# Z2PackDev/TBmodels

Hardware: AMD Instinct MI355X
Metric: k-points/sec (H(k)+eig) at N_orb=64, N_R=4096 (higher is better)
Workload: dtype f64; 1 GPU; cfg2: dense N_orb=64 N_R=4096, 100000 random k-points per GPU, eigenval (H(k)+eig); kpoints_per_gpu=100000, collective=none, rccl_ranks=0, eigensolver=auto

## Files before the change

### include/tbk.h

```cpp
#ifndef TBK_H
#define TBK_H

#include <stdint.h>

#ifdef __cplusplus
extern "C" {
#endif

typedef struct tbk_model tbk_model;
typedef struct tbk_kdotp tbk_kdotp;
typedef struct tbk_comm tbk_comm;

typedef enum tbk_status {
    TBK_OK = 0,
    TBK_ERR_ARGUMENT = 1,
    TBK_ERR_DEVICE = 2,
    TBK_ERR_MEMORY = 3,
    TBK_ERR_NOT_FINITE = 4,
    TBK_ERR_NO_CONVERGENCE = 5
} tbk_status;

enum { TBK_EIG_AUTO = 0, TBK_EIG_WAVE = 1, TBK_EIG_ROCSOLVER = 2 };
enum {
    TBK_OPT_EIGENSOLVER = 1,
    TBK_OPT_K_CHUNK = 2,
    TBK_OPT_TIMING = 3,
    TBK_OPT_FOLD = 4
};

const char* tbk_version(void);
const char* tbk_last_error(void);
int tbk_device_count(int* count);


int tbk_model_create_dense(int device, int dim, int n_orb, int64_t n_r, const int32_t* R,
                           const double* hop, tbk_model** out);

int tbk_model_create_csr(int device, int dim, int n_orb, int64_t n_r, const int32_t* R,
                         const int64_t* r_ptr, const int32_t* row, const int32_t* col,
                         const double* val, tbk_model** out);

void tbk_model_destroy(tbk_model* m);
int tbk_model_set_option(tbk_model* m, int option, int64_t value);
int tbk_model_info(const tbk_model* m, int* device, int* dim, int* n_orb, int64_t* n_r,
                   int* is_sparse, int64_t* staged_bytes);
enum { TBK_CNT_EIGENVAL_CALLS = 0, TBK_CNT_FOLDED_CALLS = 1, TBK_CNT_FOLDED_KPOINTS = 2,
       TBK_CNT_LIBRARY_CALLS = 3,
       TBK_CNT_COUNT = 4 };
int tbk_model_counter(tbk_model* m, int counter, int64_t* value);


int tbk_hamilton(tbk_model* m, const double* k, int64_t nk, int convention, const double* pos,
                 double* H_out);

int tbk_eigenval(tbk_model* m, const double* k, int64_t nk, double* E_out);

int tbk_eigenval_multi(tbk_model* const* handles, int n_handles, const double* k, int64_t nk, double* E_out);
int tbk_hamilton_multi(tbk_model* const* handles, int n_handles, const double* k, int64_t nk, int convention,
                       const double* pos, double* H_out);

int tbk_hamilton_device(tbk_model* m, const double* d_k, int64_t nk, int convention,
                        const double* d_pos, double* d_H);
int tbk_eigenval_device(tbk_model* m, const double* d_k, int64_t nk, double* d_E);
int tbk_eigenval_device_hint(tbk_model* m, const double* d_k, const double* h_k, int64_t nk, double* d_E);
int tbk_eigenval_check(tbk_model* m);
int tbk_synchronize(tbk_model* m);

enum { TBK_REDUCE_AUTO = 0, TBK_REDUCE_ONE_STAGE = 1, TBK_REDUCE_TWO_STAGE = 2 };
int tbk_tridiagonal_reduce(int device, int n_orb, int64_t nk, const double* H, int method, double* d, double* e,
                           double* H_reduced);

int tbk_reduce_standalone(int device, int n_orb, int64_t nk, int reps, double* us_per_matrix);

int tbk_kdotp_create(int device, int dim, int n_orb, int64_t n_p, const int32_t* powers,
                     const double* coeffs, tbk_kdotp** out);
void tbk_kdotp_destroy(tbk_kdotp* m);
int tbk_kdotp_hamilton(tbk_kdotp* m, const double* k, int64_t nk, double* H_out);
int tbk_kdotp_eigenval(tbk_kdotp* m, const double* k, int64_t nk, double* E_out);
int tbk_kdotp_eigenval_multi(tbk_kdotp* const* handles, int n_handles, const double* k, int64_t nk, double* E_out);
int tbk_kdotp_hamilton_multi(tbk_kdotp* const* handles, int n_handles, const double* k, int64_t nk, double* H_out);

int tbk_kdotp_coefficients(tbk_model* m, const double* k0, int64_t n_p, const int32_t* powers,
                           const double* prefactor, double* coeffs_out);

int tbk_device_malloc(int device, int64_t bytes, void** d_ptr);
int tbk_device_free(int device, void* d_ptr);
int tbk_memcpy_h2d(int device, void* d_dst, const void* h_src, int64_t bytes);
int tbk_memcpy_d2h(int device, void* h_dst, const void* d_src, int64_t bytes);
int tbk_device_mem_info(int device, int64_t* free_bytes, int64_t* total_bytes);

enum { TBK_T_PHASE = 0, TBK_T_HK = 1, TBK_T_EIG = 2, TBK_T_QL = 3, TBK_T_COUNT = 4 };
int tbk_get_timing(tbk_model* m, double* ms, int64_t* launches, int reset);

int tbk_comm_unique_id(void* id128);
int tbk_comm_create(int device, int world_size, int rank, const void* id128, tbk_comm** out);
void tbk_comm_destroy(tbk_comm* c);
int tbk_comm_ranks(tbk_comm* c, int* count, int* rank);
int tbk_comm_allgather_f64(tbk_comm* c, tbk_model* m, const double* d_send, double* d_recv,
                           int64_t count);
int tbk_comm_allgather_f64_overlapped(tbk_comm* c, tbk_model* m, const double* d_send, double* d_recv,
                                      int64_t count, int slot);
int tbk_comm_wait_slot(tbk_comm* c, tbk_model* m, int slot);
int tbk_comm_synchronize(tbk_comm* c);
int tbk_comm_agree(tbk_comm* c, int status, double* verdict);
int tbk_comm_prepare_gather(tbk_comm* c, int n_orb, int64_t per);

int tbk_eigenval_device_gather(tbk_comm* c, tbk_model* m, const double* d_k, const double* h_k, int64_t nk, int64_t per,
                               int host_status, double* d_all, double* d_status_all);

int tbk_mfma_f64_peak(int device, double* tflops);

#ifdef __cplusplus
}
#endif
#endif
```

### tbmodels_amd/csrc/tbk_api.hip

```cpp

#include <algorithm>
#include <cmath>
#include <cstdarg>
#include <cstdlib>
#include <cstring>
#include <dlfcn.h>
#include <functional>
#include <new>
#include <vector>

#include "tbk_internal.h"

static thread_local char g_err[1024] = "";

void tbk_set_error(const char* fmt, ...) {
    va_list ap;
    va_start(ap, fmt);
    vsnprintf(g_err, sizeof(g_err), fmt, ap);
    va_end(ap);
}

extern "C" const char* tbk_last_error(void) { return g_err; }
extern "C" const char* tbk_version(void) { return "tbk 0.1 (gfx950)"; }

extern "C" int tbk_device_count(int* count) {
    TBK_ARG(count != nullptr, "count is NULL");
    int n = 0;
    hipError_t e = hipGetDeviceCount(&n);
    if (e != hipSuccess) {
        (void)hipGetLastError();
        n = 0;
    }
    *count = n;
    return TBK_OK;
}

int DevBuf::reserve(size_t want) {
    if (want <= bytes) return TBK_OK;
    release();
    const size_t rounded = (want + (size_t(1) << 20) - 1) & ~((size_t(1) << 20) - 1);
    TBK_HIP(hipMalloc(&ptr, rounded));
    bytes = rounded;
    return TBK_OK;
}

void DevBuf::release() {
    if (ptr) (void)hipFree(ptr);
    ptr = nullptr;
    bytes = 0;
}

namespace {
struct RoctxApi {
    int (*push)(const char*) = nullptr;
    int (*pop)() = nullptr;
};
const RoctxApi& roctx_api() {
    static const RoctxApi api = [] {
        RoctxApi a;
        for (const char* name : {"librocprofiler-sdk-roctx.so", "librocprofiler-sdk-roctx.so.1", "libroctx64.so"}) {
            void* h = dlopen(name, RTLD_LAZY | RTLD_GLOBAL);
            if (!h) continue;
            a.push = reinterpret_cast<int (*)(const char*)>(dlsym(h, "roctxRangePushA"));
            a.pop = reinterpret_cast<int (*)()>(dlsym(h, "roctxRangePop"));
            if (a.push && a.pop) break;
            a.push = nullptr;
            a.pop = nullptr;
        }
        return a;
    }();
    return api;
}
const char* const kStageNames[TBK_T_COUNT] = {"tbk:phase_rows", "tbk:hk_contraction", "tbk:tridiag_reduction",
                                              "tbk:tridiag_eigenvalues"};
}

void tbk_range_push(const char* name) {
    const RoctxApi& api = roctx_api();
    if (api.push) (void)api.push(name);
}

void tbk_range_pop() {
    const RoctxApi& api = roctx_api();
    if (api.pop) (void)api.pop();
}

StageTimer::StageTimer(tbk_model* m_, int stage, hipStream_t s)
    : m(m_), on(m_->timing), stream(s ? s : m_->stream) {
    ev.stage = stage;
    if (on) {
        if (hipEventCreate(&ev.start) != hipSuccess || hipEventCreate(&ev.stop) != hipSuccess) {
            on = false;
            return;
        }
        tbk_range_push(kStageNames[stage]);
        (void)hipEventRecord(ev.start, stream);
    }
}

StageTimer::~StageTimer() {
    if (on) {
        (void)hipEventRecord(ev.stop, stream);
        tbk_range_pop();
        m->events.push_back(ev);
    }
}

static inline int64_t round_up(int64_t x, int64_t q) { return (x + q - 1) / q * q; }

static int require_device(int device) {
    int n = 0;
    if (hipGetDeviceCount(&n) != hipSuccess || n == 0) {
        (void)hipGetLastError();
        tbk_set_error("no HIP device visible: libtbk has no CPU path");
        return TBK_ERR_DEVICE;
    }
    if (device < 0 || device >= n) {
        tbk_set_error("device %d out of range (have %d)", device, n);
        return TBK_ERR_ARGUMENT;
    }
    TBK_HIP(hipSetDevice(device));
    return TBK_OK;
}

static int create_common(int device, int dim, int n_orb, int64_t n_r, const int32_t* R,
                         int64_t k_rows_per_r, bool pair_diagonal, tbk_model** out) {
    TBK_ARG(out != nullptr, "out is NULL");
    *out = nullptr;
    TBK_ARG(dim >= 1 && dim <= TBK_MAX_DIM, "dim must be in [1, 8]");
    TBK_ARG(n_orb >= 1 && n_orb <= 32768, "n_orb must be in [1, 32768]");
    TBK_ARG(n_r >= 0 && n_r < (int64_t(1) << 28), "n_r out of range");
    TBK_ARG(n_r == 0 || R != nullptr || k_rows_per_r == 1, "R is NULL");
    TBK_CHECK(require_device(device));

    tbk_model* m = new (std::nothrow) tbk_model();
    if (!m) {
        tbk_set_error("out of host memory");
        return TBK_ERR_MEMORY;
    }
    m->device = device;
    {
        int cus = 0;
        if (hipDeviceGetAttribute(&cus, hipDeviceAttributeMultiprocessorCount, device) == hipSuccess && cus > 0) m->n_cu = cus;
    }
    m->dim = dim;
    m->n_orb = n_orb;
    m->n_r = n_r;
    m->k2 = round_up(n_r * k_rows_per_r, TBK_BK);
    m->n_r_pad = m->k2 / k_rows_per_r;
    m->ncol = (int)(pair_diagonal ? (int64_t)n_orb * (n_orb - 1) / 2 + (n_orb + 1) / 2 : (int64_t)n_orb * (n_orb + 1) / 2);
    m->ncol_pad = (int)round_up(m->ncol, TBK_BNP);

    int rc = TBK_OK;
    auto fail = [&](int code) {
        tbk_model_destroy(m);
        return code;
    };
#define TBK_TRY(expr)                           \
    do {                                        \
        rc = [&]() -> int {                     \
            expr;                               \
            return TBK_OK;                      \
        }();                                    \
        if (rc != TBK_OK) return fail(rc);      \
    } while (0)

    TBK_TRY(TBK_HIP(hipStreamCreateWithFlags(&m->stream, hipStreamNonBlocking)));
    TBK_TRY(TBK_HIP(hipStreamCreateWithFlags(&m->stream_eig, hipStreamNonBlocking)));
    TBK_TRY(TBK_HIP(hipStreamCreateWithFlags(&m->stream_ql, hipStreamNonBlocking)));
    for (int b = 0; b < 2; ++b) {
        TBK_TRY(TBK_HIP(hipEventCreateWithFlags(&m->ev_hk[b], hipEventDisableTiming)));
        TBK_TRY(TBK_HIP(hipEventCreateWithFlags(&m->ev_tri[b], hipEventDisableTiming)));
        TBK_TRY(TBK_HIP(hipEventCreateWithFlags(&m->ev_ql[b], hipEventDisableTiming)));
        TBK_TRY(TBK_HIP(hipEventCreateWithFlags(&m->ev_out[b], hipEventDisableTiming)));
        if (b == 0) TBK_TRY(TBK_HIP(hipEventCreateWithFlags(&m->ev_sync, hipEventDisableTiming | hipEventReleaseToSystem)));
    }
    TBK_TRY(TBK_ROCBLAS(rocblas_create_handle(&m->blas)));
    TBK_TRY(TBK_ROCBLAS(rocblas_set_stream(m->blas, m->stream)));
    TBK_TRY(TBK_CHECK(m->ws_flag.reserve(2 * sizeof(int))));
    TBK_TRY(TBK_HIP(hipMemsetAsync(m->ws_flag.ptr, 0, 2 * sizeof(int), m->stream)));
    m->h_stage_bytes = std::max<size_t>(size_t(320) << 10,
                                        n_orb <= 1024 ? (size_t)n_orb * n_orb * 16 + (size_t)n_orb * dim * 8 + (size_t(64) << 10) : 0);
    if (hipHostMalloc(&m->h_stage, m->h_stage_bytes, hipHostMallocNonCoherent) != hipSuccess) {
        (void)hipGetLastError();
        m->h_stage = nullptr;
        m->h_stage_bytes = 0;
    }

    {
        std::vector<int32_t> colmap((size_t)m->ncol_pad, -1);
        size_t e = 0;
        for (int i = 0; i < n_orb; ++i) {
            if (!pair_diagonal)
                colmap[e++] = (int32_t)((i << 16) | i);
            else if (i % 2 == 0)
                colmap[e++] = i + 1 < n_orb ? (int32_t)((i << 16) | TBK_SLOT_PAIR | (i + 1)) : (int32_t)((i << 16) | i);
            for (int j = i + 1; j < n_orb; ++j) colmap[e++] = (int32_t)((i << 16) | j);
        }
        TBK_TRY(TBK_HIP(hipMalloc((void**)&m->d_colmap, colmap.size() * sizeof(int32_t))));
        TBK_TRY(TBK_HIP(hipMemcpy(m->d_colmap, colmap.data(), colmap.size() * sizeof(int32_t),
                                  hipMemcpyHostToDevice)));
        m->staged_bytes += (int64_t)(colmap.size() * sizeof(int32_t));
    }
    if (n_r > 0 && R != nullptr && k_rows_per_r == 2) m->h_R.assign(R, R + (size_t)n_r * dim);
    if (m->n_r_pad > 0 && R != nullptr) {
        std::vector<int32_t> r_pad((size_t)m->n_r_pad * dim, 0);
        std::memcpy(r_pad.data(), R, (size_t)n_r * dim * sizeof(int32_t));
        TBK_TRY(TBK_HIP(hipMalloc((void**)&m->d_R, r_pad.size() * sizeof(int32_t))));
        TBK_TRY(TBK_HIP(hipMemcpy(m->d_R, r_pad.data(), r_pad.size() * sizeof(int32_t),
                                  hipMemcpyHostToDevice)));
        m->staged_bytes += (int64_t)(r_pad.size() * sizeof(int32_t));
    }
#undef TBK_TRY
    *out = m;
    return TBK_OK;
}

extern "C" int tbk_model_create_dense(int device, int dim, int n_orb, int64_t n_r, const int32_t* R,
                                      const double* hop, tbk_model** out) {
    TBK_ARG(out != nullptr, "out is NULL");
    *out = nullptr;
    TBK_ARG(n_r == 0 || hop != nullptr, "hop is NULL");
    tbk_model* m = nullptr;
    TBK_CHECK(create_common(device, dim, n_orb, n_r, R, 2, true, &m));
    m->sparse = false;
    int rc = TBK_OK;
    double* d_raw = nullptr;
    const size_t raw_bytes = (size_t)n_r * n_orb * n_orb * 2 * sizeof(double);
    rc = [&]() -> int {
        if (raw_bytes) {
            TBK_HIP(hipMalloc((void**)&d_raw, raw_bytes));
            TBK_HIP(hipMemcpyAsync(d_raw, hop, raw_bytes, hipMemcpyHostToDevice, m->stream));
        }
        TBK_CHECK(tbk_stage_dense(m, d_raw));
        TBK_HIP(hipStreamSynchronize(m->stream));
        return TBK_OK;
    }();
    if (d_raw) (void)hipFree(d_raw);
    if (rc != TBK_OK) {
        tbk_model_destroy(m);
        return rc;
    }
    *out = m;
    return TBK_OK;
}

extern "C" int tbk_model_create_csr(int device, int dim, int n_orb, int64_t n_r, const int32_t* R,
                                    const int64_t* r_ptr, const int32_t* row, const int32_t* col,
                                    const double* val, tbk_model** out) {
    TBK_ARG(out != nullptr, "out is NULL");
    *out = nullptr;
    TBK_ARG(n_r >= 0, "n_r out of range");
    TBK_ARG(n_r == 0 || r_ptr != nullptr, "r_ptr is NULL");
    const int64_t nnz = n_r > 0 ? r_ptr[n_r] : 0;
    TBK_ARG(n_r == 0 || r_ptr[0] == 0, "r_ptr[0] must be 0");
    TBK_ARG(nnz >= 0, "negative nnz");
    TBK_ARG(nnz == 0 || (row && col && val), "row/col/val is NULL");
    for (int64_t r = 0; r < n_r; ++r) TBK_ARG(r_ptr[r] <= r_ptr[r + 1], "r_ptr not monotone");
    for (int64_t t = 0; t < nnz; ++t)
        TBK_ARG(row[t] >= 0 && row[t] < n_orb && col[t] >= 0 && col[t] < n_orb,
                "row/col index out of range");

    tbk_model* m = nullptr;
    TBK_CHECK(create_common(device, dim, n_orb, n_r, R, 2, false, &m));
    m->sparse = true;

    auto packed_index = [n_orb](int i, int j) -> int64_t {
        return (int64_t)i * n_orb - (int64_t)i * (i - 1) / 2 + (j - i);
    };
    std::vector<int64_t> cptr((size_t)m->ncol + 1, 0);
    for (int64_t t = 0; t < nnz; ++t) {
        const int i = std::min(row[t], col[t]), j = std::max(row[t], col[t]);
        cptr[(size_t)packed_index(i, j) + 1]++;
    }
    for (int e = 0; e < m->ncol; ++e) cptr[(size_t)e + 1] += cptr[(size_t)e];
    std::vector<int32_t> rec_r((size_t)nnz);
    std::vector<double> rec_v((size_t)nnz * 2);
    {
        std::vector<int64_t> cursor(cptr.begin(), cptr.end() - 1);
        for (int64_t r = 0; r < n_r; ++r)
            for (int64_t t = r_ptr[r]; t < r_ptr[r + 1]; ++t) {
                const int i = row[t], j = col[t];
                const int kind = (i == j) ? 2 : (i < j ? 0 : 1);
                const int64_t e = packed_index(std::min(i, j), std::max(i, j));
                const int64_t slot = cursor[(size_t)e]++;
                rec_r[(size_t)slot] = (int32_t)((kind << 28) | (int32_t)r);
                rec_v[(size_t)slot * 2] = val[2 * t];
                rec_v[(size_t)slot * 2 + 1] = val[2 * t + 1];
            }
    }
    m->nnz_rec = nnz;
    int rc = [&]() -> int {
        TBK_HIP(hipMalloc((void**)&m->d_cptr, cptr.size() * sizeof(int64_t)));
        TBK_HIP(hipMemcpy(m->d_cptr, cptr.data(), cptr.size() * sizeof(int64_t), hipMemcpyHostToDevice));
        m->staged_bytes += (int64_t)(cptr.size() * sizeof(int64_t));
        if (nnz > 0) {
            TBK_HIP(hipMalloc((void**)&m->d_rec_r, (size_t)nnz * sizeof(int32_t)));
            TBK_HIP(hipMalloc((void**)&m->d_rec_v, (size_t)nnz * 2 * sizeof(double)));
            TBK_HIP(hipMemcpy(m->d_rec_r, rec_r.data(), (size_t)nnz * sizeof(int32_t), hipMemcpyHostToDevice));
            TBK_HIP(hipMemcpy(m->d_rec_v, rec_v.data(), (size_t)nnz * 2 * sizeof(double), hipMemcpyHostToDevice));
            m->staged_bytes += nnz * (int64_t)(sizeof(int32_t) + 2 * sizeof(double));
            const int kt = tbk_csr_tile_kpoints(n_r);
            if (kt > 0) {
                std::vector<int64_t> sptr;
                std::vector<int32_t> srec_r;
                std::vector<double> srec_v;
                tbk_csr_schedule(m->ncol, kt, cptr, rec_r, rec_v, sptr, srec_r, srec_v);
                m->sched_steps = sptr.back();
                auto upload = [&](void** dst, const void* src, size_t bytes) -> int {
                    TBK_HIP(hipMalloc(dst, std::max<size_t>(bytes, 8)));
                    if (bytes) TBK_HIP(hipMemcpy(*dst, src, bytes, hipMemcpyHostToDevice));
                    m->staged_bytes += (int64_t)bytes;
                    return TBK_OK;
                };
                TBK_CHECK(upload((void**)&m->d_sptr, sptr.data(), sptr.size() * sizeof(int64_t)));
                TBK_CHECK(upload((void**)&m->d_srec_r, srec_r.data(), srec_r.size() * sizeof(int32_t)));
                TBK_CHECK(upload((void**)&m->d_srec_v, srec_v.data(), srec_v.size() * sizeof(double)));
                m->sched_kt = kt;
            }
        }
        return TBK_OK;
    }();
    if (rc != TBK_OK) {
        tbk_model_destroy(m);
        return rc;
    }
    *out = m;
    return TBK_OK;
}

extern "C" void tbk_model_destroy(tbk_model* m) {
    if (!m) return;
    (void)hipSetDevice(m->device);
    hipStream_t streams[] = {m->stream, m->stream_eig, m->stream_ql, m->stream_xl[0], m->stream_xl[1], m->stream_xl[2]};
    for (hipStream_t st : streams)
        if (st) (void)hipStreamSynchronize(st);
    for (hipEvent_t e : m->ev_xl)
        if (e) (void)hipEventDestroy(e);
    for (int b = 0; b < 2; ++b) {
        if (m->ev_hk[b]) (void)hipEventDestroy(m->ev_hk[b]);
        if (m->ev_tri[b]) (void)hipEventDestroy(m->ev_tri[b]);
        if (m->ev_ql[b]) (void)hipEventDestroy(m->ev_ql[b]);
        if (m->ev_out[b]) (void)hipEventDestroy(m->ev_out[b]);
        if (b == 0 && m->ev_sync) (void)hipEventDestroy(m->ev_sync);
    }
    for (auto& ev : m->events) {
        (void)hipEventDestroy(ev.start);
        (void)hipEventDestroy(ev.stop);
    }
    if (m->blas) (void)rocblas_destroy_handle(m->blas);
    if (m->h_stage) (void)hipHostFree(m->h_stage);
    for (hipStream_t st : streams)
        if (st) (void)hipStreamDestroy(st);
    void* ptrs[] = {m->d_R, m->d_colmap, m->d_B, m->d_cptr, m->d_rec_r, m->d_rec_v, m->d_powers, m->d_sptr, m->d_srec_r, m->d_srec_v};
    for (void* p : ptrs)
        if (p) (void)hipFree(p);
    DevBuf* bufs[] = {&m->ws_phase, &m->ws_H, &m->ws_E,   &m->ws_E2,
                      &m->ws_info,  &m->ws_k, &m->ws_pos, &m->ws_out, &m->ws_out2, &m->ws_flag, &m->ws_orb, &m->ws_part, &m->ws_kfold, &m->ws_kline, &m->ws_band, &m->ws_bandmat[0], &m->ws_bandmat[1], &m->ws_H2, &m->ws_xl, &m->ws_posraw};
    for (DevBuf* b : bufs) b->release();
    tbk_fold_release(m);
    delete m;
}

extern "C" int tbk_model_set_option(tbk_model* m, int option, int64_t value) {
    TBK_ARG(m != nullptr, "model is NULL");
    TBK_LOCK(m);
    switch (option) {
        case TBK_OPT_EIGENSOLVER:
            TBK_ARG(value >= TBK_EIG_AUTO && value <= TBK_EIG_ROCSOLVER, "unknown eigensolver");
            m->eigensolver = (int)value;
            return TBK_OK;
        case TBK_OPT_K_CHUNK:
            TBK_ARG(value >= 0, "k chunk must be >= 0");
            m->k_chunk = value;
            return TBK_OK;
        case TBK_OPT_TIMING:
            m->timing = value != 0;
            return TBK_OK;
        case TBK_OPT_FOLD:
            m->fold_enabled = value != 0;
            return TBK_OK;
        default:
            tbk_set_error("unknown option %d", option);
            return TBK_ERR_ARGUMENT;
    }
}

extern "C" int tbk_model_info(const tbk_model* m, int* device, int* dim, int* n_orb, int64_t* n_r,
                              int* is_sparse, int64_t* staged_bytes) {
    TBK_ARG(m != nullptr, "model is NULL");
    if (device) *device = m->device;
    if (dim) *dim = m->dim;
    if (n_orb) *n_orb = m->n_orb;
    if (n_r) *n_r = m->n_r;
    if (is_sparse) *is_sparse = m->sparse ? 1 : 0;
    if (staged_bytes) *staged_bytes = m->staged_bytes;
    return TBK_OK;
}

static int64_t choose_chunk(tbk_model* m, int64_t nk, bool with_eig) {
    if (nk <= TBK_BM) return TBK_BM;
    const int64_t n = m->n_orb;
    int64_t per_k = m->k2 * 8 + (with_eig ? n * n * 16 + (int64_t)tbk_eig_scratch_per_k(m) : 0);
    if (per_k < 64) per_k = 64;
    size_t free_b = 0, total_b = 0;
    if (hipMemGetInfo(&free_b, &total_b) != hipSuccess) free_b = size_t(8) << 30;
    free_b += m->ws_H.bytes + m->ws_H2.bytes + m->ws_phase.bytes + m->ws_band.bytes + m->ws_bandmat[0].bytes + m->ws_bandmat[1].bytes +
              m->ws_E.bytes + m->ws_xl.bytes;
    const bool mid = n > 64 && n <= 256;
    int64_t budget = std::min<int64_t>((int64_t)(free_b / 4), int64_t(mid ? 64 : n > 64 ? 24 : 6) << 30);
    int64_t chunk = budget / per_k / TBK_BM * TBK_BM;
    int64_t cap = mid ? 131072 : 32768;
    if (n < 64) cap *= std::min<int64_t>(32, (64 / n) * (64 / n));
    chunk = std::max<int64_t>(TBK_BM, std::min<int64_t>(chunk, cap));
    if (m->k_chunk > 0) chunk = round_up(m->k_chunk, TBK_BM);
    else if (chunk >= 4096) chunk = chunk / 4096 * 4096;
    return std::min(chunk, round_up(nk, TBK_BM));
}

static inline int64_t phase_ld(int64_t nk) { return round_up(nk, TBK_BM); }

static int fill_rows(tbk_model* m, const double* d_k, int64_t nk, int64_t nk_pad, double* d_A) {
    if (m->kdotp)
        return tbk_launch_monomials(m->stream, m->d_powers, m->dim, m->n_r, m->k2, d_k, nk, nk_pad, d_A);
    return tbk_launch_phase(m, d_k, nk, nk_pad, d_A);
}

static int build_h(tbk_model* m, const double* d_A, int64_t nk, int64_t nk_pad, int mode,
                   int convention, const double* d_k, const double* d_pos, double* d_H) {
    if (m->sparse)
        return tbk_launch_hk_csr(m, d_A, nk, nk_pad, mode, convention, d_k, d_pos, d_H);
    return tbk_launch_hk_dense(m, d_A, nk, nk_pad, mode, convention, d_k, d_pos, d_H);
}

extern "C" int tbk_hamilton_device(tbk_model* m, const double* d_k, int64_t nk, int convention,
                                   const double* d_pos, double* d_H) {
    TBK_ARG(m != nullptr, "model is NULL");
    TBK_LOCK(m);
    TBK_ARG(convention == 1 || convention == 2, "convention must be 1 or 2");
    TBK_ARG(nk >= 0, "nk < 0");
    if (nk == 0) return TBK_OK;
    TBK_ARG(d_k && d_H, "k / H is NULL");
    TBK_ARG(convention == 2 || d_pos != nullptr, "convention 1 needs pos");
    TBK_HIP(hipSetDevice(m->device));
    const int64_t chunk = choose_chunk(m, nk, false);
    const size_t nn2 = (size_t)m->n_orb * m->n_orb * 2;
    for (int64_t c0 = 0; c0 < nk; c0 += chunk) {
        const int64_t nkc = std::min(chunk, nk - c0);
        const int64_t nk_pad = phase_ld(nkc);
        TBK_CHECK(m->ws_phase.reserve((size_t)std::max<int64_t>(m->k2, 1) * nk_pad * sizeof(double)));
        double* d_A = m->ws_phase.as<double>();
        const double* kc = d_k + c0 * m->dim;
        const bool own_rows = tbk_hk_inline_phases(m, nkc);
        if (!own_rows) TBK_CHECK(fill_rows(m, kc, nkc, nk_pad, d_A));
        const double* d_orb = nullptr;
        const bool inline_orb = m->h_k_inline != nullptr && m->d_pos_inline != nullptr && nk == 1 && own_rows;
        if (convention == 1 && !inline_orb) {
            TBK_CHECK(m->ws_orb.reserve((size_t)nkc * m->n_orb * 2 * sizeof(double)));
            TBK_CHECK(tbk_launch_orbital_phases(m, kc, d_pos, nkc, m->ws_orb.as<double>()));
            d_orb = m->ws_orb.as<double>();
        }
        TBK_CHECK(build_h(m, own_rows ? nullptr : d_A, nkc, nk_pad, HK_FULL, convention, kc, d_orb, d_H + (size_t)c0 * nn2));
    }
    return TBK_OK;
}

constexpr int64_t TBK_SMALL_CALL = 4096;
constexpr int64_t TBK_SMALL_CALL_PER_ORBITAL = 768;

static int launch_tridiag_eigenvalues(tbk_model* m, hipStream_t s, double* d_de, int64_t nk, double* d_E,
                                      bool beside_ql = false, bool small_call = false, const void* d_band = nullptr) {
    if (d_band) TBK_CHECK(tbk_launch_band_chase(m, s, d_band, nk, d_de));
    if (tbk_eig_small_supported(m->n_orb) && !small_call) return tbk_launch_ql(m, s, d_de, nk, d_E, beside_ql);
    return tbk_launch_bisect(m, s, d_de, nk, d_E);
}

static std::vector<int64_t> chunk_schedule(tbk_model* m, int64_t nk, int64_t chunk) {
    std::vector<int64_t> out;
    const int64_t unit = 4096;
    if (!tbk_eig_small_supported(m->n_orb) || m->k_chunk > 0 || chunk < 2 * unit || nk < 3 * unit) {
        for (int64_t c0 = 0; c0 < nk; c0 += chunk) out.push_back(std::min(chunk, nk - c0));
        return out;
    }
    const int64_t last = unit + nk % unit;
    int64_t rest = nk - last;
    const int64_t n_big = (rest + chunk - 1) / chunk;
    for (int64_t i = 0; i < n_big; ++i) {
        const int64_t share = round_up((rest + (n_big - i) - 1) / (n_big - i), unit);
        const int64_t take = std::min(std::min(share, chunk), rest);
        out.push_back(take);
        rest -= take;
    }
    out.push_back(last);
    return out;
}

using HBuilder = std::function<int(int64_t c0, int64_t nkc, double* d_H)>;

static std::vector<int64_t> run_schedule(const std::vector<int64_t>& runs, int64_t chunk) {
    std::vector<int64_t> out;
    int64_t cur = 0;
    for (size_t r = 0; r + 1 < runs.size(); ++r) {
        int64_t len = runs[r + 1] - runs[r];
        if (cur > 0 && cur + len > chunk) {
            out.push_back(cur);
            cur = 0;
        }
        while (len > chunk) {
            out.push_back(chunk);
            len -= chunk;
        }
        cur += len;
    }
    if (cur > 0) out.push_back(cur);
    return out;
}

static int eigenval_wave_pipeline(tbk_model* m, const double* d_k, int64_t nk, double* d_E, const HBuilder* builder = nullptr,
                                  const std::vector<int64_t>* runs = nullptr) {
    int64_t rows_ready_for = -1;
    const auto prepare_rows = [&](int64_t c0, int64_t nkc) -> int {
        if (tbk_hk_inline_phases(m, nkc)) return TBK_OK;
        const int64_t nk_pad = phase_ld(nkc);
        TBK_CHECK(m->ws_phase.reserve((size_t)std::max<int64_t>(m->k2, 1) * nk_pad * sizeof(double)));
        TBK_CHECK(fill_rows(m, d_k + c0 * m->dim, nkc, nk_pad, m->ws_phase.as<double>()));
        rows_ready_for = c0;
        return TBK_OK;
    };
    const HBuilder direct = [&](int64_t c0, int64_t nkc, double* d_H) -> int {
        const int64_t nk_pad = phase_ld(nkc);
        const double* kc = d_k + c0 * m->dim;
        if (tbk_hk_inline_phases(m, nkc)) return build_h(m, nullptr, nkc, nk_pad, HK_TRI, 2, kc, nullptr, d_H);
        if (rows_ready_for != c0) TBK_CHECK(prepare_rows(c0, nkc));
        return build_h(m, m->ws_phase.as<double>(), nkc, nk_pad, HK_TRI, 2, kc, nullptr, d_H);
    };
    const HBuilder& build = builder ? *builder : direct;
    const int64_t chunk = choose_chunk(m, nk, true);
    const size_t n = (size_t)m->n_orb;
    const size_t nn2 = n * n * 2;
    DevBuf* debuf[2] = {&m->ws_E, &m->ws_E2};
    const std::vector<int64_t> sched =
        (runs != nullptr && m->k_chunk == 0 && nk > chunk) ? run_schedule(*runs, chunk) : chunk_schedule(m, nk, chunk);
    const int64_t n_chunks = (int64_t)sched.size();
    const int64_t max_chunk = *std::max_element(sched.begin(), sched.end());
    const bool small_call = nk <= std::max<int64_t>(TBK_SMALL_CALL, TBK_SMALL_CALL_PER_ORBITAL * (int64_t)m->n_orb);
    TBK_CHECK(m->ws_H.reserve((size_t)max_chunk * nn2 * sizeof(double)));
    for (int b = 0; b < (n_chunks > 1 ? 2 : 1); ++b)
        TBK_CHECK(debuf[b]->reserve((size_t)max_chunk * n * 2 * sizeof(double)));
    double* d_H = m->ws_H.as<double>();
    const bool h_overlap = n_chunks > 2 && builder != nullptr && tbk_eig_small_supported(m->n_orb);
    double* d_Hbuf[2] = {d_H, d_H};
    if (h_overlap) {
        TBK_CHECK(m->ws_H2.reserve((size_t)max_chunk * nn2 * sizeof(double)));
        d_Hbuf[1] = m->ws_H2.as<double>();
    }
    const bool two_stage = !tbk_eig_small_supported(m->n_orb) && tbk_eig_two_stage(m) && n_chunks > 1 && !tbk_band_fused(m->n_orb);
    if (two_stage) {
        TBK_CHECK(m->ws_band.reserve((size_t)max_chunk * tbk_band_scratch_per_matrix(m->n_orb)));
        for (int b = 0; b < 2; ++b) TBK_CHECK(m->ws_bandmat[b].reserve((size_t)max_chunk * tbk_band_bytes_per_matrix(m->n_orb)));
        TBK_CHECK(tbk_band_xl_reserve(m, max_chunk));
    }
    if (n_chunks == 1) {
        double* d_de = debuf[0]->as<double>();
        TBK_CHECK(build(0, nk, d_H));
        if (tbk_eig_small_supported(m->n_orb))
            TBK_CHECK(tbk_launch_tridiag(m, m->stream, d_H, nk, d_de));
        else
            TBK_CHECK(tbk_launch_tridiag_stream(m, m->stream, d_H, nk, d_de));
        TBK_CHECK(launch_tridiag_eigenvalues(m, m->stream, d_de, nk, d_E, false, small_call));
        if (m->chunk_done) {
            TBK_HIP(hipEventRecord(m->ev_ql[0], m->stream));
            TBK_CHECK(m->chunk_done(0, nk, m->ev_ql[0]));
        }
        return TBK_OK;
    }
    int64_t prev_c0 = 0, prev_nkc = 0, c0 = 0;
    for (int64_t c = 0; c < n_chunks; ++c) {
        const int b = (int)(c & 1);
        const int64_t nkc = sched[c];
        double* d_de = debuf[b]->as<double>();
        d_H = d_Hbuf[b];
        if (c >= 1) {
            if (!builder) TBK_CHECK(prepare_rows(c0, nkc));
            if (!h_overlap)
                TBK_HIP(hipStreamWaitEvent(m->stream, m->ev_tri[b ^ 1], 0));
            else if (c >= 2)
                TBK_HIP(hipStreamWaitEvent(m->stream, m->ev_tri[b], 0));
            if (c >= 2 && !h_overlap) TBK_HIP(hipStreamWaitEvent(m->stream, m->ev_ql[b], 0));
        }
        TBK_CHECK(build(c0, nkc, d_H));
        TBK_HIP(hipEventRecord(m->ev_hk[b], m->stream));

        TBK_HIP(hipStreamWaitEvent(m->stream_eig, m->ev_hk[b], 0));
        if (c >= 2 && h_overlap) TBK_HIP(hipStreamWaitEvent(m->stream_eig, m->ev_ql[b], 0));
        if (tbk_eig_small_supported(m->n_orb))
            TBK_CHECK(tbk_launch_tridiag(m, m->stream_eig, d_H, nkc, d_de));
        else if (two_stage)
            TBK_CHECK(tbk_launch_band_reduce(m, m->stream_eig, d_H, nkc, m->ws_band.ptr, m->ws_bandmat[b].ptr));
        else
            TBK_CHECK(tbk_launch_tridiag_stream(m, m->stream_eig, d_H, nkc, d_de));
        TBK_HIP(hipEventRecord(m->ev_tri[b], m->stream_eig));

        if (c >= 1) {
            TBK_HIP(hipStreamWaitEvent(m->stream_ql, m->ev_hk[b], 0));
            if (h_overlap) TBK_HIP(hipStreamWaitEvent(m->stream_ql, m->ev_tri[b ^ 1], 0));
            TBK_CHECK(launch_tridiag_eigenvalues(m, m->stream_ql, debuf[b ^ 1]->as<double>(), prev_nkc,
                                                 d_E + (size_t)prev_c0 * n, false, small_call,
                                                 two_stage ? m->ws_bandmat[b ^ 1].ptr : nullptr));
            TBK_HIP(hipEventRecord(m->ev_ql[b ^ 1], m->stream_ql));
            if (m->chunk_done) TBK_CHECK(m->chunk_done(prev_c0, prev_nkc, m->ev_ql[b ^ 1]));
        }
        prev_c0 = c0;
        prev_nkc = nkc;
        c0 += nkc;
    }
    {
        const int b = (int)((n_chunks - 1) & 1);
        TBK_CHECK(launch_tridiag_eigenvalues(m, m->stream_eig, debuf[b]->as<double>(), prev_nkc,
                                             d_E + (size_t)prev_c0 * n, n_chunks > 1,
                                             small_call || n_chunks > 1, two_stage ? m->ws_bandmat[b].ptr : nullptr));
        TBK_HIP(hipEventRecord(m->ev_ql[b], m->stream_eig));
        if (m->chunk_done) TBK_CHECK(m->chunk_done(prev_c0, prev_nkc, m->ev_ql[b]));
    }
    for (int b = 0; b < (n_chunks > 1 ? 2 : 1); ++b) TBK_HIP(hipStreamWaitEvent(m->stream, m->ev_ql[b], 0));
    TBK_HIP(hipStreamWaitEvent(m->stream, m->ev_tri[(n_chunks - 1) & 1], 0));
    return TBK_OK;
}

static int eigenval_folded(tbk_model* m, const double* d_k, const double* h_k, int64_t nk, double* d_E, bool* done) {
    *done = false;
    if (!m->fold_enabled || m->sparse || m->kdotp || m->dim < 2 || m->n_r < 64 || nk < 1024) return TBK_OK;
    if (h_k == nullptr) return TBK_OK;
    std::vector<int64_t> runs;
    const int f = tbk_fold_choose(m, h_k, nk, runs);
    if (f < 0) return TBK_OK;
    const int dim = m->dim;
    TBK_CHECK(m->ws_kfold.reserve((size_t)nk * (dim - 1) * sizeof(double)));
    double* d_k2 = m->ws_kfold.as<double>();
    TBK_CHECK(tbk_fold_drop_component(m, d_k, dim, f, nk, d_k2));
    const size_t nn2 = (size_t)m->n_orb * m->n_orb * 2;
    const int64_t n_runs = (int64_t)runs.size() - 1;
    const int group = tbk_fold_group_size();
    int64_t group_lo = -1;
    tbk_fold_plan_t& plan1 = m->fold[f];
    std::vector<int> reduced;
    for (int d = 0; d < dim; ++d)
        if (d != f) reduced.push_back(d);

    auto piece_plane = [&](int64_t lo, int64_t hi, double* d_Hp) -> int {
        const int64_t len = hi - lo, nk_pad = phase_ld(len);
        TBK_CHECK(m->ws_phase.reserve((size_t)std::max<int64_t>(m->k2, 1) * nk_pad * sizeof(double)));
        TBK_CHECK(fill_rows(m, d_k2 + lo * (dim - 1), len, nk_pad, m->ws_phase.as<double>()));
        return build_h(m, m->ws_phase.as<double>(), len, nk_pad, HK_TRI, 2, d_k2 + lo * (dim - 1), nullptr, d_Hp);
    };

    struct LineInfo {
        bool ok = false;
        int e2 = -1;
        int64_t L = 0;
        int64_t body = 0;
        int64_t n_lines = 0;
    };
    const int dim1 = dim - 1;
    const int line_cap = 512;
    auto same_line = [&](int64_t a0, int64_t b0, int64_t L, int e2) {
        for (int64_t t = 0; t < L; ++t)
            for (int e = 0; e < dim1; ++e)
                if (e != e2 && h_k[(a0 + t) * dim + reduced[e]] != h_k[(b0 + t) * dim + reduced[e]]) return false;
        return true;
    };
    auto analyse = [&](int64_t lo, int64_t hi) -> LineInfo {
        LineInfo li;
        if (dim1 < 2 || hi - lo < 512) return li;
        int e2 = -1;
        int64_t best_changes = hi - lo;
        for (int e = 0; e < dim1; ++e) {
            int64_t changes = 0;
            for (int64_t i = lo + 1; i < hi; ++i) changes += h_k[i * dim + reduced[e]] != h_k[(i - 1) * dim + reduced[e]];
            if (changes < best_changes) {
                best_changes = changes;
                e2 = e;
            }
        }
        if (e2 < 0 || best_changes < 4) return li;
        const int c2 = reduced[e2];
        std::vector<int64_t> sb(1, lo);
        for (int64_t i = lo + 1; i < hi; ++i)
            if (h_k[i * dim + c2] != h_k[(i - 1) * dim + c2]) sb.push_back(i);
        sb.push_back(hi);
        const size_t n_sub = sb.size() - 1;
        if (n_sub < 6) return li;
        const int64_t L = sb[2] - sb[1];
        if (L < 8 || L > TBK_BM) return li;
        size_t first = (sb[1] - sb[0] == L && same_line(sb[0], sb[1], L, e2)) ? 0 : 1, last = first;
        while (last < n_sub && sb[last + 1] - sb[last] == L && same_line(sb[first], sb[last], L, e2)) ++last;
        li.n_lines = (int64_t)(last - first);
        if (li.n_lines < 4) return li;
        li.ok = true;
        li.e2 = e2;
        li.L = L;
        li.body = sb[first];
        return li;
    };
    auto fold_body = [&](tbk_fold_plan_t& plan2, const LineInfo& li, int64_t a0, int64_t n, int slot0) -> int {
        return tbk_fold_lines(m, plan2, d_k2 + a0 * dim1 + li.e2, li.L * dim1, (int)n, slot0);
    };
    auto contract_lines = [&](tbk_fold_plan_t& plan2, const LineInfo& li, int64_t a0, int64_t n, double* d_Hp) -> int {
        const int64_t row_len = (int64_t)m->ncol_pad * 2;
        tbk_fold_saved_t saved2;
        TBK_CHECK(tbk_fold_enter(m, plan2, 0, saved2));
        int rc = m->ws_kline.reserve((size_t)li.L * std::max(dim1 - 1, 1) * sizeof(double));
        if (rc == TBK_OK) rc = tbk_fold_drop_component(m, d_k2 + a0 * dim1, dim1, li.e2, li.L, m->ws_kline.as<double>());
        if (rc == TBK_OK) rc = m->ws_phase.reserve((size_t)std::max<int64_t>(m->k2, 1) * TBK_BM * sizeof(double));
        if (rc == TBK_OK) rc = fill_rows(m, m->ws_kline.as<double>(), li.L, TBK_BM, m->ws_phase.as<double>());
        if (rc == TBK_OK)
            rc = tbk_launch_hk_dense_lines(m, m->ws_phase.as<double>(), n, (int)li.L, plan2.k2 * row_len, d_Hp);
        tbk_fold_leave(m, saved2);
        return rc;
    };

    auto piece = [&](int64_t lo, int64_t hi, double* d_Hp) -> int {
        const LineInfo li = analyse(lo, hi);
        if (!li.ok) return piece_plane(lo, hi, d_Hp);
        tbk_fold_plan_t* plan2 = nullptr;
        TBK_CHECK(tbk_fold_subplan(m, plan1, li.e2, line_cap, &plan2));
        if (!plan2 || plan2->n_rho * 3 > plan1.n_rho) return piece_plane(lo, hi, d_Hp);

        if (li.body > lo) TBK_CHECK(piece_plane(lo, li.body, d_Hp));
        for (int64_t l0 = 0; l0 < li.n_lines; l0 += line_cap) {
            const int64_t nl = std::min<int64_t>(line_cap, li.n_lines - l0);
            const int64_t a0 = li.body + l0 * li.L;
            TBK_CHECK(fold_body(*plan2, li, a0, nl, 0));
            TBK_CHECK(contract_lines(*plan2, li, a0, nl, d_Hp + (size_t)(a0 - lo) * nn2));
        }
        const int64_t body_end = li.body + li.n_lines * li.L;
        if (body_end < hi) TBK_CHECK(piece_plane(body_end, hi, d_Hp + (size_t)(body_end - lo) * nn2));
        return TBK_OK;
    };

    auto enter_run = [&](size_t r, tbk_fold_saved_t& saved) -> int {
        if (group_lo < 0 || (int64_t)r < group_lo || (int64_t)r >= group_lo + group) {
            group_lo = (int64_t)r;
            const int n_g = (int)std::min<int64_t>(group, n_runs - group_lo);
            double kf[64];
            for (int g = 0; g < n_g; ++g) kf[g] = h_k[runs[(size_t)(group_lo + g)] * dim + f];
            TBK_CHECK(tbk_fold_group(m, plan1, kf, n_g, 0));
        }
        return tbk_fold_enter(m, plan1, (int)((int64_t)r - group_lo), saved);
    };
    auto batched = [&](int64_t c0, int64_t nkc, double* d_H, bool* done) -> int {
        *done = false;
        const size_t r0 = (size_t)(std::upper_bound(runs.begin(), runs.end(), c0) - runs.begin()) - 1;
        if (runs[r0] != c0) return TBK_OK;
        size_t r1 = r0;
        while (r1 + 1 < runs.size() && runs[r1 + 1] <= c0 + nkc) ++r1;
        if (r1 - r0 < 2 || runs[r1] != c0 + nkc) return TBK_OK;
        const LineInfo li0 = analyse(runs[r0], runs[r0 + 1]);
        if (!li0.ok || li0.body != runs[r0] || li0.body + li0.n_lines * li0.L != runs[r0 + 1]) return TBK_OK;
        int64_t total = li0.n_lines;
        for (size_t r = r0 + 1; r < r1; ++r) {
            const LineInfo li = analyse(runs[r], runs[r + 1]);
            if (!li.ok || li.e2 != li0.e2 || li.L != li0.L || li.body != runs[r] ||
                li.body + li.n_lines * li.L != runs[r + 1] || !same_line(runs[r0], runs[r], li0.L, li0.e2))
                return TBK_OK;
            total += li.n_lines;
        }
        if (total > line_cap) return TBK_OK;
        tbk_fold_plan_t* plan2 = nullptr;
        TBK_CHECK(tbk_fold_subplan(m, plan1, li0.e2, line_cap, &plan2));
        if (!plan2 || plan2->n_rho * 3 > plan1.n_rho) return TBK_OK;
        int slot = 0;
        for (size_t r = r0; r < r1; ++r) {
            tbk_fold_saved_t saved;
            TBK_CHECK(enter_run(r, saved));
            const int64_t n = (runs[r + 1] - runs[r]) / li0.L;
            const int rc = fold_body(*plan2, li0, runs[r], n, slot);
            tbk_fold_leave(m, saved);
            TBK_CHECK(rc);
            slot += (int)n;
        }
        {
            tbk_fold_saved_t saved;
            TBK_CHECK(enter_run(r1 - 1, saved));
            const int rc = contract_lines(*plan2, li0, c0, total, d_H);
            tbk_fold_leave(m, saved);
            TBK_CHECK(rc);
        }
        *done = true;
        return TBK_OK;
    };

    const HBuilder folded = [&](int64_t c0, int64_t nkc, double* d_H) -> int {
        {
            bool done = false;
            TBK_CHECK(batched(c0, nkc, d_H, &done));
            if (done) return TBK_OK;
        }
        size_t r = (size_t)(std::upper_bound(runs.begin(), runs.end(), c0) - runs.begin()) - 1;
        for (int64_t lo = c0; lo < c0 + nkc; ++r) {
            const int64_t hi = std::min(runs[r + 1], c0 + nkc);
            tbk_fold_saved_t saved;
            TBK_CHECK(enter_run(r, saved));
            const int rc = piece(lo, hi, d_H + (size_t)(lo - c0) * nn2);
            tbk_fold_leave(m, saved);
            TBK_CHECK(rc);
            lo = hi;
        }
        return TBK_OK;
    };
    TBK_CHECK(eigenval_wave_pipeline(m, d_k, nk, d_E, &folded, &runs));
    m->counters[TBK_CNT_FOLDED_CALLS] += 1;
    m->counters[TBK_CNT_FOLDED_KPOINTS] += nk;
    *done = true;
    return TBK_OK;
}

static bool eigenval_own_solvers(const tbk_model* m) {
    return m->eigensolver != TBK_EIG_ROCSOLVER &&
           (tbk_eig_small_supported(m->n_orb) || (m->eigensolver == TBK_EIG_AUTO && tbk_eig_stream_supported(m->n_orb)));
}

static int eigenval_device_solve(tbk_model* m, const double* d_k, const double* h_k, int64_t nk, double* d_E) {
    TBK_ARG(m != nullptr, "model is NULL");
    TBK_LOCK(m);
    TBK_ARG(nk >= 0, "nk < 0");
    if (nk == 0) return TBK_OK;
    TBK_ARG(d_k && d_E, "k / E is NULL");
    TBK_HIP(hipSetDevice(m->device));
    m->call_nk = nk;
    m->counters[TBK_CNT_EIGENVAL_CALLS] += 1;
    if (m->eigensolver == TBK_EIG_WAVE && !tbk_eig_small_supported(m->n_orb)) {
        tbk_set_error("TBK_EIG_WAVE handles n_orb <= 64 only (n_orb = %d)", m->n_orb);
        return TBK_ERR_ARGUMENT;
    }
    if (eigenval_own_solvers(m)) {
        bool done = false;
        TBK_CHECK(eigenval_folded(m, d_k, h_k, nk, d_E, &done));
        if (done) return TBK_OK;
        return eigenval_wave_pipeline(m, d_k, nk, d_E);
    }

    int64_t chunk = choose_chunk(m, nk, true);
    const size_t nn2 = (size_t)m->n_orb * m->n_orb * 2;
    chunk = std::max<int64_t>(1, std::min<int64_t>(chunk, (int64_t(1) << 29) / std::max<int64_t>(1, (int64_t)m->n_orb * m->n_orb)));
    m->counters[TBK_CNT_LIBRARY_CALLS] += 1;
    for (int64_t c0 = 0; c0 < nk; c0 += chunk) {
        const int64_t nkc = std::min(chunk, nk - c0);
        const int64_t nk_pad = phase_ld(nkc);
        TBK_CHECK(m->ws_phase.reserve((size_t)std::max<int64_t>(m->k2, 1) * nk_pad * sizeof(double)));
        TBK_CHECK(m->ws_H.reserve((size_t)nkc * nn2 * sizeof(double)));
        double* d_A = m->ws_phase.as<double>();
        double* d_H = m->ws_H.as<double>();
        const double* kc = d_k + c0 * m->dim;
        TBK_CHECK(fill_rows(m, kc, nkc, nk_pad, d_A));
        TBK_CHECK(build_h(m, d_A, nkc, nk_pad, HK_TRI, 2, kc, nullptr, d_H));
        TBK_CHECK(tbk_eig_batched(m, d_H, nkc, d_E + (size_t)c0 * m->n_orb));
    }
    return TBK_OK;
}

__global__ void __launch_bounds__(256) flag_nonfinite_kernel(const double* __restrict__ E, int64_t total, int* __restrict__ flag) {
    bool bad = false;
    for (int64_t i = (int64_t)blockIdx.x * 256 + threadIdx.x; i < total; i += (int64_t)gridDim.x * 256) bad |= !isfinite(E[i]);
    if (__any(bad) && (threadIdx.x & 63) == 0) atomicAdd(flag, 1);
}

static int eigenval_device_impl(tbk_model* m, const double* d_k, const double* h_k, int64_t nk, double* d_E) {
    TBK_CHECK(eigenval_device_solve(m, d_k, h_k, nk, d_E));
    const bool own_solvers = m != nullptr && eigenval_own_solvers(m);
    if (nk > 0 && m != nullptr && !own_solvers) {
        const int64_t total = nk * m->n_orb;
        const unsigned blocks = (unsigned)std::min<int64_t>((total + 255) / 256, 8 * 1024);
        hipLaunchKernelGGL(flag_nonfinite_kernel, dim3(blocks), dim3(256), 0, m->stream, d_E, total, m->ws_flag.as<int>() + 1);
        TBK_HIP(hipGetLastError());
    }
    return TBK_OK;
}

extern "C" int tbk_eigenval_device(tbk_model* m, const double* d_k, int64_t nk, double* d_E) {
    return eigenval_device_impl(m, d_k, nullptr, nk, d_E);
}

extern "C" int tbk_eigenval_device_hint(tbk_model* m, const double* d_k, const double* h_k, int64_t nk, double* d_E) {
    return eigenval_device_impl(m, d_k, h_k, nk, d_E);
}

extern "C" int tbk_model_counter(tbk_model* m, int counter, int64_t* value) {
    TBK_ARG(m != nullptr && value != nullptr, "model / value is NULL");
    TBK_ARG(counter >= 0 && counter < TBK_CNT_COUNT, "unknown counter");
    TBK_LOCK(m);
    *value = m->counters[counter];
    return TBK_OK;
}

static int wait_main_stream(tbk_model* m) {
    TBK_HIP(hipEventRecord(m->ev_sync, m->stream));
    TBK_HIP(hipEventSynchronize(m->ev_sync));
    return TBK_OK;
}

extern "C" int tbk_synchronize(tbk_model* m) {
    TBK_ARG(m != nullptr, "model is NULL");
    TBK_LOCK(m);
    TBK_HIP(hipSetDevice(m->device));
    return wait_main_stream(m);
}

extern "C" int tbk_eigenval_check(tbk_model* m) {
    TBK_ARG(m != nullptr, "model is NULL");
    TBK_LOCK(m);
    TBK_HIP(hipSetDevice(m->device));
    int flag[2] = {0, 0};
    TBK_HIP(hipMemcpyAsync(flag, m->ws_flag.ptr, sizeof(flag), hipMemcpyDeviceToHost, m->stream));
    TBK_HIP(hipMemsetAsync(m->ws_flag.ptr, 0, sizeof(flag), m->stream));
    TBK_CHECK(wait_main_stream(m));
    if (flag[1] != 0) {
        tbk_set_error("array must not contain infs or NaNs");
        return TBK_ERR_NOT_FINITE;
    }
    if (flag[0] != 0) {
        tbk_set_error("eigensolver did not converge for %d matrices", flag[0]);
        return TBK_ERR_NO_CONVERGENCE;
    }
    return TBK_OK;
}

extern "C" int tbk_hamilton(tbk_model* m, const double* k, int64_t nk, int convention,
                            const double* pos, double* H_out) {
    TBK_ARG(m != nullptr, "model is NULL");
    TBK_LOCK(m);
    TBK_ARG(convention == 1 || convention == 2, "convention must be 1 or 2");
    TBK_ARG(nk >= 0, "nk < 0");
    if (nk == 0) return TBK_OK;
    TBK_ARG(k && H_out, "k / H is NULL");
    TBK_ARG(convention == 2 || pos != nullptr, "convention 1 needs pos");
    TBK_HIP(hipSetDevice(m->device));
    const size_t nn2 = (size_t)m->n_orb * m->n_orb * 2;
    {
        const size_t k_bytes = (size_t)nk * m->dim * sizeof(double), h_bytes = (size_t)nk * nn2 * sizeof(double);
        const size_t p_bytes = convention == 1 ? (size_t)m->n_orb * m->dim * sizeof(double) : 0;
        const size_t h_off = (k_bytes + p_bytes + 63) / 64 * 64;
        if (m->h_stage != nullptr && h_off + h_bytes <= m->h_stage_bytes) {
            char* st = static_cast<char*>(m->h_stage);
            TBK_CHECK(m->ws_k.reserve(k_bytes));
            TBK_CHECK(m->ws_out.reserve(h_bytes));
            const bool inline_k = nk == 1 && !m->sparse && !m->kdotp && tbk_hk_inline_phases(m, 1);
            const double* d_pos = nullptr;
            if (inline_k) {
                if (convention == 1) {
                    const size_t n_pos = (size_t)m->n_orb * m->dim;
                    if (m->pos_cache.size() != n_pos || std::memcmp(m->pos_cache.data(), pos, p_bytes) != 0) {
                        TBK_CHECK(m->ws_posraw.reserve(p_bytes));
                        std::memcpy(st + k_bytes, pos, p_bytes);
                        TBK_HIP(hipMemcpyAsync(m->ws_posraw.ptr, st + k_bytes, p_bytes, hipMemcpyHostToDevice, m->stream));
                        m->pos_cache.assign(pos, pos + n_pos);
                    }
                    m->d_pos_inline = m->ws_posraw.as<double>();
                    d_pos = m->d_pos_inline;
                }
                m->h_k_inline = k;
            } else {
                std::memcpy(st, k, k_bytes);
                TBK_HIP(hipMemcpyAsync(m->ws_k.ptr, st, k_bytes, hipMemcpyHostToDevice, m->stream));
                if (convention == 1) {
                    TBK_CHECK(m->ws_pos.reserve(p_bytes));
                    std::memcpy(st + k_bytes, pos, p_bytes);
                    TBK_HIP(hipMemcpyAsync(m->ws_pos.ptr, st + k_bytes, p_bytes, hipMemcpyHostToDevice, m->stream));
                    d_pos = m->ws_pos.as<double>();
                }
            }
            constexpr size_t ZERO_COPY_MAX = size_t(1) << 20;
            const bool direct = h_bytes <= ZERO_COPY_MAX;
            double* d_out = direct ? reinterpret_cast<double*>(st + h_off) : m->ws_out.as<double>();
            const int rc_inline = tbk_hamilton_device(m, m->ws_k.as<double>(), nk, convention, d_pos, d_out);
            m->h_k_inline = nullptr;
            m->d_pos_inline = nullptr;
            TBK_CHECK(rc_inline);
            if (!direct) TBK_HIP(hipMemcpyAsync(st + h_off, m->ws_out.ptr, h_bytes, hipMemcpyDeviceToHost, m->stream));
            TBK_CHECK(wait_main_stream(m));
            std::memcpy(H_out, st + h_off, h_bytes);
            return TBK_OK;
        }
    }
    const size_t total_bytes = (size_t)nk * nn2 * sizeof(double);
    const size_t chunk_bytes = std::min<size_t>(size_t(128) << 20, std::max<size_t>(size_t(16) << 20, total_bytes / 4));
    int64_t out_chunk = std::max<int64_t>(1, (int64_t)(chunk_bytes / (nn2 * sizeof(double))));
    out_chunk = std::min(out_chunk, nk);
    const int64_t n_chunks = (nk + out_chunk - 1) / out_chunk;
    TBK_CHECK(m->ws_k.reserve((size_t)nk * m->dim * sizeof(double)));
    TBK_HIP(hipMemcpyAsync(m->ws_k.ptr, k, (size_t)nk * m->dim * sizeof(double), hipMemcpyHostToDevice, m->stream));
    const double* d_pos = nullptr;
    if (convention == 1) {
        TBK_CHECK(m->ws_pos.reserve((size_t)m->n_orb * m->dim * sizeof(double)));
        TBK_HIP(hipMemcpyAsync(m->ws_pos.ptr, pos, (size_t)m->n_orb * m->dim * sizeof(double),
                               hipMemcpyHostToDevice, m->stream));
        d_pos = m->ws_pos.as<double>();
    }
    DevBuf* obuf[2] = {&m->ws_out, &m->ws_out2};
    for (int b = 0; b < (n_chunks > 1 ? 2 : 1); ++b) TBK_CHECK(obuf[b]->reserve((size_t)out_chunk * nn2 * sizeof(double)));
    auto compute = [&](int64_t c) -> int {
        const int64_t c0 = c * out_chunk, nkc = std::min(out_chunk, nk - c0);
        TBK_CHECK(tbk_hamilton_device(m, m->ws_k.as<double>() + c0 * m->dim, nkc, convention, d_pos, obuf[c & 1]->as<double>()));
        TBK_HIP(hipEventRecord(m->ev_out[c & 1], m->stream));
        return TBK_OK;
    };
    TBK_CHECK(compute(0));
    for (int64_t c = 0; c < n_chunks; ++c) {
        const int64_t c0 = c * out_chunk, nkc = std::min(out_chunk, nk - c0);
        if (c + 1 < n_chunks) TBK_CHECK(compute(c + 1));
        TBK_HIP(hipEventSynchronize(m->ev_out[c & 1]));
        TBK_HIP(hipMemcpy(H_out + (size_t)c0 * nn2, obuf[c & 1]->ptr, (size_t)nkc * nn2 * sizeof(double), hipMemcpyDeviceToHost));
    }
    return wait_main_stream(m);
}

__global__ void __launch_bounds__(256) export_small_kernel(const double* __restrict__ E, int64_t count, const int* __restrict__ flag,
                                                           double* __restrict__ host_E, int* __restrict__ host_flag) {
    for (int64_t i = (int64_t)blockIdx.x * 256 + threadIdx.x; i < count; i += (int64_t)gridDim.x * 256) host_E[i] = E[i];
    if (blockIdx.x == 0 && threadIdx.x < 2) host_flag[threadIdx.x] = flag[threadIdx.x];
}

extern "C" int tbk_eigenval(tbk_model* m, const double* k, int64_t nk, double* E_out) {
    TBK_ARG(m != nullptr, "model is NULL");
    TBK_LOCK(m);
    TBK_ARG(nk >= 0, "nk < 0");
    if (nk == 0) return TBK_OK;
    TBK_ARG(k && E_out, "k / E is NULL");
    TBK_HIP(hipSetDevice(m->device));
    const size_t k_bytes = (size_t)nk * m->dim * sizeof(double), e_bytes = (size_t)nk * m->n_orb * sizeof(double);
    TBK_CHECK(m->ws_k.reserve(k_bytes));
    TBK_CHECK(m->ws_out.reserve(e_bytes));
    const size_t e_off = (k_bytes + 63) / 64 * 64;
    if (m->h_stage != nullptr && e_off + e_bytes + 16 <= m->h_stage_bytes) {
        char* st = static_cast<char*>(m->h_stage);
        int* flag = reinterpret_cast<int*>(st + e_off + e_bytes);
        const bool inline_k = nk == 1 && !m->sparse && !m->kdotp && eigenval_own_solvers(m) && tbk_hk_inline_phases(m, 1);
        if (inline_k) {
            m->h_k_inline = k;
        } else {
            std::memcpy(st, k, k_bytes);
            TBK_HIP(hipMemcpyAsync(m->ws_k.ptr, st, k_bytes, hipMemcpyHostToDevice, m->stream));
        }
        const int rc_inline = eigenval_device_impl(m, m->ws_k.as<double>(), k, nk, m->ws_out.as<double>());
        m->h_k_inline = nullptr;
        TBK_CHECK(rc_inline);
        {
            const int64_t count = nk * m->n_orb;
            const unsigned blocks = (unsigned)std::min<int64_t>((count + 255) / 256, 64);
            hipLaunchKernelGGL(export_small_kernel, dim3(blocks), dim3(256), 0, m->stream, m->ws_out.as<double>(), count,
                               m->ws_flag.as<int>(), reinterpret_cast<double*>(st + e_off), flag);
            TBK_HIP(hipGetLastError());
        }
        TBK_CHECK(wait_main_stream(m));
        std::memcpy(E_out, st + e_off, e_bytes);
        if (flag[0] != 0 || flag[1] != 0) return tbk_eigenval_check(m);
        return TBK_OK;
    }
    TBK_HIP(hipMemcpyAsync(m->ws_k.ptr, k, k_bytes, hipMemcpyHostToDevice, m->stream));
    TBK_CHECK(eigenval_device_impl(m, m->ws_k.as<double>(), k, nk, m->ws_out.as<double>()));
    TBK_HIP(hipMemcpyAsync(E_out, m->ws_out.ptr, e_bytes, hipMemcpyDeviceToHost, m->stream));
    return tbk_eigenval_check(m);
}

extern "C" int tbk_tridiagonal_reduce(int device, int n_orb, int64_t nk, const double* H, int method, double* d, double* e,
                                      double* H_reduced) {
    TBK_ARG(nk >= 0, "nk < 0");
    TBK_ARG(n_orb >= 1 && (n_orb <= 64 || tbk_eig_stream_supported(n_orb)),
            "n_orb must be in [1, 4096] (larger matrices go through rocSOLVER as a whole)");
    TBK_ARG(method >= TBK_REDUCE_AUTO && method <= TBK_REDUCE_TWO_STAGE, "unknown reduction method");
    TBK_ARG(method != TBK_REDUCE_TWO_STAGE || tbk_eig_band_supported(n_orb), "the two-stage reduction handles 64 < n_orb <= 4096");
    TBK_ARG(method != TBK_REDUCE_ONE_STAGE || n_orb <= 512, "the one-stage reduction handles n_orb <= 512");
    if (nk == 0) return TBK_OK;
    TBK_ARG(H && d && e, "H / d / e is NULL");
    tbk_model* m = nullptr;
    TBK_CHECK(create_common(device, 1, n_orb, 0, nullptr, 2, false, &m));
    const size_t n = (size_t)n_orb, mat_bytes = n * n * 2 * sizeof(double);
    int rc = [&]() -> int {
        TBK_LOCK(m);
        m->call_nk = nk;
        TBK_CHECK(m->ws_H.reserve((size_t)nk * mat_bytes));
        TBK_CHECK(m->ws_E.reserve((size_t)nk * n * 2 * sizeof(double)));
        TBK_HIP(hipMemcpyAsync(m->ws_H.ptr, H, (size_t)nk * mat_bytes, hipMemcpyHostToDevice, m->stream));
        if (tbk_eig_small_supported(n_orb))
            TBK_CHECK(tbk_launch_tridiag(m, m->stream, m->ws_H.as<double>(), nk, m->ws_E.as<double>()));
        else
            TBK_CHECK(tbk_launch_tridiag_stream(m, m->stream, m->ws_H.as<double>(), nk, m->ws_E.as<double>(), method));
        TBK_HIP(hipMemcpyAsync(d, m->ws_E.ptr, (size_t)nk * n * sizeof(double), hipMemcpyDeviceToHost, m->stream));
        TBK_HIP(hipMemcpyAsync(e, m->ws_E.as<double>() + (size_t)nk * n, (size_t)nk * n * sizeof(double), hipMemcpyDeviceToHost,
                               m->stream));
        if (H_reduced)
            TBK_HIP(hipMemcpyAsync(H_reduced, m->ws_H.ptr, (size_t)nk * mat_bytes, hipMemcpyDeviceToHost, m->stream));
        TBK_HIP(hipStreamSynchronize(m->stream));
        return TBK_OK;
    }();
    tbk_model_destroy(m);
    return rc;
}

__global__ void __launch_bounds__(256) random_hermitian_kernel(double* __restrict__ H, int n, int64_t nk) {
    const int64_t total = nk * (int64_t)n * n;
    for (int64_t t = (int64_t)blockIdx.x * 256 + threadIdx.x; t < total; t += (int64_t)gridDim.x * 256) {
        const int64_t mat = t / ((int64_t)n * n);
        const int r = (int)((t / n) % n), c = (int)(t % n);
        const int i = r < c ? r : c, j = r < c ? c : r;
        uint64_t x = (uint64_t)mat * 0x9E3779B97F4A7C15ull + (uint64_t)i * 0xBF58476D1CE4E5B9ull + (uint64_t)j * 0x94D049BB133111EBull + 1;
        x ^= x >> 30; x *= 0xBF58476D1CE4E5B9ull; x ^= x >> 27; x *= 0x94D049BB133111EBull; x ^= x >> 31;
        const double re = (double)(int64_t)(x >> 11) * (1.0 / 9007199254740992.0) - 0.5;
        x ^= x >> 29; x *= 0x9E3779B97F4A7C15ull; x ^= x >> 32;
        const double im = (double)(int64_t)(x >> 11) * (1.0 / 9007199254740992.0) - 0.5;
        H[2 * t] = re;
        H[2 * t + 1] = i == j ? 0.0 : (r < c ? im : -im);
    }
}

extern "C" int tbk_reduce_standalone(int device, int n_orb, int64_t nk, int reps, double* us_per_matrix) {
    TBK_ARG(us_per_matrix != nullptr, "us_per_matrix is NULL");
    TBK_ARG(nk >= 1 && reps >= 1, "nk / reps < 1");
    TBK_ARG(n_orb >= 1 && (n_orb <= 64 || tbk_eig_stream_supported(n_orb)), "n_orb must be in [1, 4096]");
    for (int q = 0; q < 3; ++q) us_per_matrix[q] = 0.0;
    tbk_model* m = nullptr;
    TBK_CHECK(create_common(device, 1, n_orb, 0, nullptr, 2, false, &m));
    const size_t n = (size_t)n_orb, mat_bytes = n * n * 2 * sizeof(double);
    DevBuf pristine;
    hipEvent_t ev[2] = {nullptr, nullptr};
    int rc = [&]() -> int {
        TBK_LOCK(m);
        m->call_nk = nk;
        TBK_CHECK(pristine.reserve((size_t)nk * mat_bytes));
        TBK_CHECK(m->ws_H.reserve((size_t)nk * mat_bytes));
        TBK_CHECK(m->ws_E.reserve((size_t)nk * n * 2 * sizeof(double)));
        TBK_HIP(hipEventCreate(&ev[0]));
        TBK_HIP(hipEventCreate(&ev[1]));
        hipLaunchKernelGGL(random_hermitian_kernel, dim3(4096), dim3(256), 0, m->stream, pristine.as<double>(), n_orb, nk);
        TBK_HIP(hipGetLastError());
        const bool band = !tbk_eig_small_supported(n_orb) && tbk_eig_two_stage(m);
        if (band) {
            TBK_CHECK(m->ws_band.reserve((size_t)nk * tbk_band_scratch_per_matrix(n_orb)));
            TBK_CHECK(m->ws_bandmat[0].reserve((size_t)nk * tbk_band_bytes_per_matrix(n_orb)));
        }
        for (int what = 0; what < (band ? 3 : 1); ++what) {
            float sum = 0.0f;
            for (int r = 0; r <= reps; ++r) {
                if (what != 2)
                    TBK_HIP(hipMemcpyAsync(m->ws_H.ptr, pristine.ptr, (size_t)nk * mat_bytes, hipMemcpyDeviceToDevice, m->stream));
                TBK_HIP(hipEventRecord(ev[0], m->stream));
                if (what == 0) {
                    if (tbk_eig_small_supported(n_orb))
                        TBK_CHECK(tbk_launch_tridiag(m, m->stream, m->ws_H.as<double>(), nk, m->ws_E.as<double>()));
                    else
                        TBK_CHECK(tbk_launch_tridiag_stream(m, m->stream, m->ws_H.as<double>(), nk, m->ws_E.as<double>(), TBK_REDUCE_AUTO));
                } else if (what == 1) {
                    TBK_CHECK(tbk_launch_band_reduce(m, m->stream, m->ws_H.as<double>(), nk, m->ws_band.ptr, m->ws_bandmat[0].ptr));
                } else {
                    TBK_CHECK(tbk_launch_band_chase(m, m->stream, m->ws_bandmat[0].ptr, nk, m->ws_E.as<double>()));
                }
                TBK_HIP(hipEventRecord(ev[1], m->stream));
                TBK_HIP(hipEventSynchronize(ev[1]));
                float ms = 0.0f;
                TBK_HIP(hipEventElapsedTime(&ms, ev[0], ev[1]));
                if (r > 0) sum += ms;
            }
            us_per_matrix[what] = (double)sum / reps * 1e3 / (double)nk;
        }
        return TBK_OK;
    }();
    for (auto& e : ev)
        if (e) (void)hipEventDestroy(e);
    pristine.release();
    tbk_model_destroy(m);
    return rc;
}

extern "C" int tbk_kdotp_create(int device, int dim, int n_orb, int64_t n_p, const int32_t* powers,
                                const double* coeffs, tbk_kdotp** out) {
    TBK_ARG(out != nullptr, "out is NULL");
    *out = nullptr;
    TBK_ARG(n_p == 0 || (powers && coeffs), "powers / coeffs is NULL");
    for (int64_t t = 0; t < n_p * dim; ++t) TBK_ARG(powers[t] >= 0, "negative power");
    tbk_model* m = nullptr;
    TBK_CHECK(create_common(device, dim, n_orb, n_p, nullptr, 1, false, &m));
    m->kdotp = true;
    double* d_raw = nullptr;
    const size_t raw_bytes = (size_t)n_p * n_orb * n_orb * 2 * sizeof(double);
    int rc = [&]() -> int {
        if (n_p > 0) {
            TBK_HIP(hipMalloc((void**)&m->d_powers, (size_t)n_p * dim * sizeof(int32_t)));
            TBK_HIP(hipMemcpy(m->d_powers, powers, (size_t)n_p * dim * sizeof(int32_t), hipMemcpyHostToDevice));
            TBK_HIP(hipMalloc((void**)&d_raw, raw_bytes));
            TBK_HIP(hipMemcpyAsync(d_raw, coeffs, raw_bytes, hipMemcpyHostToDevice, m->stream));
        }
        TBK_CHECK(tbk_stage_kdotp(m, d_raw));
        TBK_HIP(hipStreamSynchronize(m->stream));
        return TBK_OK;
    }();
    if (d_raw) (void)hipFree(d_raw);
    if (rc != TBK_OK) {
        tbk_model_destroy(m);
        return rc;
    }
    tbk_kdotp* kp = new (std::nothrow) tbk_kdotp();
    if (!kp) {
        tbk_model_destroy(m);
        tbk_set_error("out of host memory");
        return TBK_ERR_MEMORY;
    }
    kp->core = m;
    *out = kp;
    return TBK_OK;
}

extern "C" void tbk_kdotp_destroy(tbk_kdotp* kp) {
    if (!kp) return;
    tbk_model_destroy(kp->core);
    delete kp;
}

extern "C" int tbk_kdotp_hamilton(tbk_kdotp* kp, const double* k, int64_t nk, double* H_out) {
    TBK_ARG(kp != nullptr, "model is NULL");
    return tbk_hamilton(kp->core, k, nk, 2, nullptr, H_out);
}

extern "C" int tbk_kdotp_eigenval(tbk_kdotp* kp, const double* k, int64_t nk, double* E_out) {
    TBK_ARG(kp != nullptr, "model is NULL");
    return tbk_eigenval(kp->core, k, nk, E_out);
}

extern "C" int tbk_device_malloc(int device, int64_t bytes, void** d_ptr) {
    TBK_ARG(d_ptr != nullptr && bytes >= 0, "bad malloc arguments");
    TBK_CHECK(require_device(device));
    *d_ptr = nullptr;
    if (bytes == 0) return TBK_OK;
    TBK_HIP(hipMalloc(d_ptr, (size_t)bytes));
    return TBK_OK;
}

extern "C" int tbk_device_free(int device, void* d_ptr) {
    if (!d_ptr) return TBK_OK;
    TBK_CHECK(require_device(device));
    TBK_HIP(hipFree(d_ptr));
    return TBK_OK;
}

extern "C" int tbk_memcpy_h2d(int device, void* d_dst, const void* h_src, int64_t bytes) {
    TBK_CHECK(require_device(device));
    if (bytes > 0) {
        TBK_HIP(hipMemcpy(d_dst, h_src, (size_t)bytes, hipMemcpyHostToDevice));
        TBK_HIP(hipDeviceSynchronize());
    }
    return TBK_OK;
}

extern "C" int tbk_memcpy_d2h(int device, void* h_dst, const void* d_src, int64_t bytes) {
    TBK_CHECK(require_device(device));
    if (bytes > 0) TBK_HIP(hipMemcpy(h_dst, d_src, (size_t)bytes, hipMemcpyDeviceToHost));
    return TBK_OK;
}

extern "C" int tbk_device_mem_info(int device, int64_t* free_bytes, int64_t* total_bytes) {
    TBK_CHECK(require_device(device));
    size_t f = 0, t = 0;
    TBK_HIP(hipMemGetInfo(&f, &t));
    if (free_bytes) *free_bytes = (int64_t)f;
    if (total_bytes) *total_bytes = (int64_t)t;
    return TBK_OK;
}

extern "C" int tbk_get_timing(tbk_model* m, double* ms, int64_t* launches, int reset) {
    TBK_ARG(m != nullptr, "model is NULL");
    TBK_LOCK(m);
    TBK_HIP(hipSetDevice(m->device));
    TBK_HIP(hipStreamSynchronize(m->stream));
    TBK_HIP(hipStreamSynchronize(m->stream_eig));
    TBK_HIP(hipStreamSynchronize(m->stream_ql));
    for (auto& ev : m->events) {
        float t = 0.f;
        if (hipEventElapsedTime(&t, ev.start, ev.stop) == hipSuccess) {
            m->t_ms[ev.stage] += (double)t;
            m->t_n[ev.stage] += 1;
        }
        (void)hipEventDestroy(ev.start);
        (void)hipEventDestroy(ev.stop);
    }
    m->events.clear();
    for (int i = 0; i < TBK_T_COUNT; ++i) {
        if (ms) ms[i] = m->t_ms[i];
        if (launches) launches[i] = m->t_n[i];
        if (reset) {
            m->t_ms[i] = 0.0;
            m->t_n[i] = 0;
        }
    }
    return TBK_OK;
}

extern "C" int tbk_mfma_f64_peak(int device, double* tflops) {
    TBK_ARG(tflops != nullptr, "tflops is NULL");
    TBK_CHECK(require_device(device));
    return tbk_run_mfma_f64_peak(tflops);
}
```

### tbmodels_amd/csrc/tbk_hk_dense.hip

```cpp

#include <algorithm>
#include <cstdlib>
#include <type_traits>

#include "tbk_internal.h"

namespace {

typedef double d4 __attribute__((ext_vector_type(4)));
typedef double d2 __attribute__((ext_vector_type(2)));
typedef __attribute__((address_space(1))) const void* gptr_t;
typedef __attribute__((address_space(3))) void* lptr_t;

constexpr int LDA = TBK_BM + 16;
constexpr int LDB = 2 * TBK_BNP + 16;
constexpr int STAGE_DOUBLES = TBK_BK * (LDA + LDB);

static_assert(TBK_BM == 128 && TBK_BNP == 64 && TBK_BK == 16, "wave decomposition is written for 128x64x16");

struct HkArgs {
    const double* A;
    const double* Bt;
    const int32_t* colmap;
    const double* kpts;
    const int32_t* R;
    int64_t n_r;
    const double* pos;
    double* H;
    int64_t k2;
    int64_t nk;
    int64_t nk_pad;
    int ncol_pad;
    int n_orb;
    int dim;
    int mt_count;
    int nt_count;
    int xcd_rows;
    double* P;
    int splits;
    int unit_grid;
    int64_t p_rows;
    int64_t a_tile_stride;
    int64_t b_tile_stride;
    int rows_per_tile;
    int block_offset;
    int p_tiles;
    int sub_splits;
    double* P2;
    double k_val[TBK_MAX_DIM];
    int k_inline;
    const double* pos_raw;
};

__device__ __forceinline__ double hk_kcomp(const HkArgs& a, int64_t kq, int d) { return a.k_inline ? a.k_val[d] : a.kpts[kq * a.dim + d]; }

template <int MODE, int CONV>
__device__ __forceinline__ void store_element(const HkArgs& a, int64_t kq, int oi, int oj, double re, double im) {
    if (CONV == 1 && oi != oj) {
        d2 ei, ej;
        if (a.k_inline) {
            double di = 0.0, dj = 0.0;
            for (int d = 0; d < a.dim; ++d) {
                di = fma(a.k_val[d], a.pos_raw[oi * a.dim + d], di);
                dj = fma(a.k_val[d], a.pos_raw[oj * a.dim + d], dj);
            }
            double sn, cs;
            sincospi(2.0 * di, &sn, &cs);
            ei = (d2){cs, sn};
            sincospi(2.0 * dj, &sn, &cs);
            ej = (d2){cs, sn};
        } else {
            ei = *reinterpret_cast<const d2*>(a.pos + ((size_t)kq * a.n_orb + oi) * 2);
            ej = *reinterpret_cast<const d2*>(a.pos + ((size_t)kq * a.n_orb + oj) * 2);
        }
        const double cs = ei[0] * ej[0] + ei[1] * ej[1], sn = ei[0] * ej[1] - ei[1] * ej[0];
        const double t = re * cs - im * sn;
        im = re * sn + im * cs;
        re = t;
    }
    double* hk = a.H + (size_t)kq * a.n_orb * a.n_orb * 2;
    *reinterpret_cast<d2*>(hk + ((size_t)oi * a.n_orb + oj) * 2) = (d2){re, im};
    if (MODE == HK_FULL && oi != oj) *reinterpret_cast<d2*>(hk + ((size_t)oj * a.n_orb + oi) * 2) = (d2){re, -im};
}

template <int MODE, int CONV>
__device__ __forceinline__ void store_slot(const HkArgs& a, int64_t kq, int32_t slot, double v0, double v1) {
    const int oi = slot >> 16, oj = slot & 0x7fff;
    if (slot & TBK_SLOT_PAIR) {
        double* hk = a.H + (size_t)kq * a.n_orb * a.n_orb * 2;
        *reinterpret_cast<d2*>(hk + ((size_t)oi * a.n_orb + oi) * 2) = (d2){v0, 0.0};
        *reinterpret_cast<d2*>(hk + ((size_t)oj * a.n_orb + oj) * 2) = (d2){v1, 0.0};
        return;
    }
    store_element<MODE, CONV>(a, kq, oi, oj, v0, v1);
}

__device__ __forceinline__ bool tile_of_block(const HkArgs& a, int b, int& mt, int& nt) {
    if (a.xcd_rows == 0) {
        nt = b % a.nt_count;
        mt = b / a.nt_count;
        return mt < a.mt_count;
    }
    const int x = b & 7;
    const int t = b >> 3;
    const int base = a.mt_count >> 3, extra = a.mt_count & 7;
    const int rows = base + (x < extra ? 1 : 0);
    if (t >= rows * a.nt_count) return false;
    const int start = x * base + (x < extra ? x : extra);
    const int full = rows / a.xcd_rows;
    const int per_group = a.xcd_rows * a.nt_count;
    int row;
    if (t < full * per_group) {
        const int g = t / per_group, r = t % per_group;
        row = g * a.xcd_rows + r % a.xcd_rows;
        nt = r / a.xcd_rows;
    } else {
        const int tt = t - full * per_group, rr = rows - full * a.xcd_rows;
        row = full * a.xcd_rows + tt % rr;
        nt = tt / rr;
    }
    mt = start + row;
    return true;
}

template <int MODE, int CONV, bool SPLIT>
__global__ void __launch_bounds__(256, 2) hk_dense_kernel(const HkArgs a) {
    extern __shared__ __attribute__((aligned(16))) double smem[];

    const int unit = (int)blockIdx.x + a.block_offset;
    const int split_y = SPLIT ? unit / a.unit_grid : 0;
    int mt_idx, nt_idx;
    if (!tile_of_block(a, SPLIT ? unit - split_y * a.unit_grid : unit, mt_idx, nt_idx)) return;

    const int tid = threadIdx.x;
    const int lane = tid & 63;
    const int wave = __builtin_amdgcn_readfirstlane(tid >> 6);
    const int wm = wave >> 1;
    const int wn = wave & 1;
    const int l15 = lane & 15;
    const int l4 = lane >> 4;

    const int64_t m0 = (int64_t)mt_idx * a.rows_per_tile;
    const int64_t n0 = (int64_t)nt_idx * TBK_BNP;

    d4 acc[4][2][2];
#pragma unroll
    for (int i = 0; i < 4; ++i)
#pragma unroll
        for (int j = 0; j < 2; ++j)
#pragma unroll
            for (int p = 0; p < 2; ++p) acc[i][j][p] = (d4){0.0, 0.0, 0.0, 0.0};

    int s_begin = 0, n_stage = (int)(a.k2 / TBK_BK);
    if (SPLIT) {
        const int per = (n_stage + a.splits - 1) / a.splits;
        s_begin = min(split_y * per, n_stage);
        n_stage = min(s_begin + per, n_stage);
        if (a.p_tiles > 0) {
            const int per2 = (n_stage - s_begin + a.sub_splits - 1) / a.sub_splits;
            s_begin = min(s_begin + (int)blockIdx.y * per2, n_stage);
            n_stage = min(s_begin + per2, n_stage);
        }
    }

    const uint32_t lane_bytes = (uint32_t)lane * 16u;
    const int64_t ldgA = a.nk_pad * (int64_t)sizeof(double);
    const int64_t ldgB = (int64_t)a.ncol_pad * 2 * (int64_t)sizeof(double);
    const char* rowA = reinterpret_cast<const char*>(a.A + (int64_t)mt_idx * a.a_tile_stride) + ((int64_t)s_begin * TBK_BK + wave) * ldgA;
    const char* rowB = reinterpret_cast<const char*>(a.Bt + (int64_t)mt_idx * a.b_tile_stride + n0 * 2) + ((int64_t)s_begin * TBK_BK + wave) * ldgB;
    auto issue_stage = [&](auto bufc) {
        constexpr int buf = decltype(bufc)::value;
        double* sA = smem + buf * STAGE_DOUBLES + wave * LDA;
        double* sB = smem + buf * STAGE_DOUBLES + TBK_BK * LDA + wave * LDB;
        uint32_t off = lane_bytes;
        asm volatile("" : "+v"(off));
#pragma unroll
        for (int i = 0; i < 4; ++i) {
            __builtin_amdgcn_global_load_lds((gptr_t)(rowA + (int64_t)(4 * i) * ldgA + off), (lptr_t)(sA + 4 * i * LDA), 16, 0, 0);
            __builtin_amdgcn_global_load_lds((gptr_t)(rowB + (int64_t)(4 * i) * ldgB + off), (lptr_t)(sB + 4 * i * LDB), 16, 0, 0);
        }
        rowA += TBK_BK * ldgA;
        rowB += TBK_BK * ldgB;
    };
    typedef __attribute__((address_space(3))) const double* lds_cptr;
    uint32_t fragA[2][TBK_BK / 4], fragB[2][TBK_BK / 4];
    {
        const uint32_t s0 = (uint32_t)(uintptr_t)(lptr_t)smem;
#pragma unroll
        for (int buf = 0; buf < 2; ++buf)
#pragma unroll
            for (int ks = 0; ks < TBK_BK / 4; ++ks) {
                fragA[buf][ks] = s0 + 8u * (uint32_t)(buf * STAGE_DOUBLES + wm * 64 + l15 + (ks * 4 + l4) * LDA);
                fragB[buf][ks] = s0 + 8u * (uint32_t)(buf * STAGE_DOUBLES + TBK_BK * LDA + wn * 64 + l15 + (ks * 4 + l4) * LDB);
                asm volatile("" : "+v"(fragA[buf][ks]), "+v"(fragB[buf][ks]));
            }
    }
    struct Frags {
        double fa[4], fb[2][2];
    };
    auto read_frags = [&](auto bufc, auto ksc) -> Frags {
        constexpr int buf = decltype(bufc)::value, ks = decltype(ksc)::value;
        const lds_cptr sA = (lds_cptr)(uintptr_t)fragA[buf][ks];
        const lds_cptr sB = (lds_cptr)(uintptr_t)fragB[buf][ks];
        Frags f;
#pragma unroll
        for (int i = 0; i < 4; ++i) f.fa[i] = sA[i * 16];
#pragma unroll
        for (int j = 0; j < 2; ++j) {
            f.fb[j][0] = sB[j * 32];
            f.fb[j][1] = sB[j * 32 + 16];
        }
        return f;
    };
    auto mfma_step = [&](const Frags& f) {
#pragma unroll
        for (int i = 0; i < 4; ++i)
#pragma unroll
            for (int j = 0; j < 2; ++j) {
                acc[i][j][0] = __builtin_amdgcn_mfma_f64_16x16x4f64(f.fa[i], f.fb[j][0], acc[i][j][0], 0, 0, 0);
                acc[i][j][1] = __builtin_amdgcn_mfma_f64_16x16x4f64(f.fa[i], f.fb[j][1], acc[i][j][1], 0, 0, 0);
            }
    };
    using buf0 = std::integral_constant<int, 0>;
    using buf1 = std::integral_constant<int, 1>;
    using ks0 = std::integral_constant<int, 0>;
    using ks1 = std::integral_constant<int, 1>;
    using ks2 = std::integral_constant<int, 2>;
    using ks3 = std::integral_constant<int, 3>;
    static_assert(TBK_BK == 16, "four K steps per stage are written out below");
    auto stage = [&](auto bufc, auto nextc, Frags& cur, bool more) {
        Frags f1 = read_frags(bufc, ks1{});
        mfma_step(cur);
        Frags f2 = read_frags(bufc, ks2{});
        mfma_step(f1);
        Frags f3 = read_frags(bufc, ks3{});
        mfma_step(f2);
        __syncthreads();
        if (more) cur = read_frags(nextc, ks0{});
        mfma_step(f3);
    };

    const int left = n_stage - s_begin;
    if (left > 0) issue_stage(buf0{});
    __syncthreads();
    Frags cur = read_frags(buf0{}, ks0{});
    for (int pair = 0; pair < (left >> 1); ++pair) {
        issue_stage(buf1{});
        stage(buf0{}, buf1{}, cur, true);
        const bool more = 2 * pair + 2 < left;
        if (more) issue_stage(buf0{});
        stage(buf1{}, buf0{}, cur, more);
    }
    if (left & 1) stage(buf0{}, buf1{}, cur, false);

#pragma unroll
    for (int j = 0; j < 2; ++j) {
        const int e = (int)n0 + (wn * 2 + j) * 16 + l15;
        const int32_t ij = a.colmap[e];
        if (ij < 0) continue;
#pragma unroll
        for (int i = 0; i < 4; ++i) {
#pragma unroll
            for (int r = 0; r < 4; ++r) {
                const int local = wm * 64 + i * 16 + l4 + 4 * r;
                const int64_t kq = m0 + local;
                if (local >= a.rows_per_tile || kq >= a.nk) continue;
                if (SPLIT) {
                    double* part =
                        a.p_tiles > 0
                            ? a.P2 + ((((size_t)blockIdx.y * a.p_tiles + blockIdx.x) * TBK_BM + local) * TBK_BNP +
                                      (wn * 2 + j) * 16 + l15) * 2
                            : a.P + (((size_t)split_y * a.p_rows + kq) * a.ncol_pad + e) * 2;
                    *reinterpret_cast<d2*>(part) = (d2){acc[i][j][0][r], acc[i][j][1][r]};
                } else {
                    store_slot<MODE, CONV>(a, kq, ij, acc[i][j][0][r], acc[i][j][1][r]);
                }
            }
        }
    }
}

constexpr int GEMV_U = 8;

template <int NKV, bool INLINE_PHASES>
__global__ void __launch_bounds__(256) hk_gemv_kernel(const HkArgs a, int strip_doubles) {
    extern __shared__ __attribute__((aligned(16))) double s_rows[];
    constexpr int U = NKV >= 32 ? 4 : GEMV_U;
    const int lane = threadIdx.x & 63;
    const int wave = __builtin_amdgcn_readfirstlane(threadIdx.x >> 6);
    const int nblk = a.ncol_pad >> 6;
    const int b = (int)blockIdx.x, n_wg = (int)gridDim.x;
    const int xcd = b & 7, per_xcd = n_wg >> 3, extra = n_wg & 7;
    const int wg = xcd * per_xcd + min(xcd, extra) + (b >> 3);
    const int task = wg * 4 + wave;
    const int sl = task / nblk, cb = task - sl * nblk;
    if (sl >= a.splits) return;
    const int64_t n_pairs = a.k2 >> 1;
    const int64_t kk0 = 2 * (sl * n_pairs / a.splits);
    const int n_rows = (int)(2 * ((sl + 1) * n_pairs / a.splits) - kk0);
    const int64_t kbase = (int64_t)blockIdx.z * NKV;
    const int nk_here = (int)min((int64_t)NKV, a.nk - kbase);
    const int64_t ld2 = a.ncol_pad;
    const d2* rows = reinterpret_cast<const d2*>(a.Bt) + kk0 * ld2 + cb * 64;
    double* strip = s_rows + wave * strip_doubles;

    d2 buf0[U], buf1[U];
    double acc[NKV][2];
#pragma unroll
    for (int q = 0; q < NKV; ++q) acc[q][0] = acc[q][1] = 0.0;

    auto fetch = [&](d2 (&buf)[U], int base) {
#pragma unroll
        for (int u = 0; u < U; ++u) {
            const int r = min(base + u, n_rows - 1);
            buf[u] = __builtin_nontemporal_load(rows + (int64_t)r * ld2 + lane);
        }
    };
    auto consume = [&](const d2 (&buf)[U], int row) {
        const double* arow = INLINE_PHASES ? strip + row * NKV : a.A + (kk0 + row) * a.nk_pad + kbase;
        const int64_t lda = INLINE_PHASES ? NKV : a.nk_pad;
#pragma unroll
        for (int u = 0; u < U; ++u) {
            if (!INLINE_PHASES && row + u >= n_rows) break;
#pragma unroll
            for (int q = 0; q < NKV; ++q) {
                const double aq = arow[u * lda + q];
                acc[q][0] = fma(aq, buf[u][0], acc[q][0]);
                acc[q][1] = fma(aq, buf[u][1], acc[q][1]);
            }
        }
    };
    fetch(buf0, 0);
    fetch(buf1, U);
    if (INLINE_PHASES) {
        for (int idx = lane; idx < ((n_rows + 15) >> 4) * 8 * NKV; idx += 64) {
            const int rr = idx / NKV, q = idx % NKV;
            const int64_t r = (kk0 >> 1) + rr;
            double sn = 0.0, cs = 0.0;
            if (q < nk_here && r < a.n_r && 2 * rr < n_rows) {
                double dot = 0.0;
                for (int d = 0; d < a.dim; ++d) dot = fma(hk_kcomp(a, kbase + q, d), (double)a.R[r * a.dim + d], dot);
                sincospi(2.0 * dot, &sn, &cs);
            }
            strip[(2 * rr) * NKV + q] = cs;
            strip[(2 * rr + 1) * NKV + q] = sn;
        }
        asm volatile("s_waitcnt lgkmcnt(0)" ::: "memory");
    }
    for (int row = 0; row < n_rows; row += 2 * U) {
        consume(buf0, row);
        __builtin_amdgcn_sched_barrier(0);
        fetch(buf0, row + 2 * U);
        __builtin_amdgcn_sched_barrier(0);
        consume(buf1, row + U);
        __builtin_amdgcn_sched_barrier(0);
        fetch(buf1, row + 3 * U);
        __builtin_amdgcn_sched_barrier(0);
    }
    const bool hi = (lane & 8) != 0;
    const int e = cb * 64 + (lane >> 4) * 16 + (lane & 7) * 2 + (hi ? 1 : 0);
#pragma unroll
    for (int q = 0; q < NKV; ++q) {
        const double got = __shfl_xor(hi ? acc[q][0] : acc[q][1], 8, 64);
        if (q < nk_here) {
            double* part = a.P + (((size_t)sl * a.p_rows + kbase + q) * a.ncol_pad + e) * 2;
            *reinterpret_cast<d2*>(part) = hi ? (d2){got, acc[q][1]} : (d2){acc[q][0], got};
        }
    }
}

template <int MODE, int CONV>
__global__ void __launch_bounds__(256) hk_tiny_kernel(const HkArgs a, int strip_doubles) {
    extern __shared__ __attribute__((aligned(16))) double s_tiny[];
    const int lane = threadIdx.x & 63;
    const int wave = __builtin_amdgcn_readfirstlane(threadIdx.x >> 6);
    const int cb = blockIdx.x;
    const int64_t n_pairs = a.k2 >> 1;
    const int64_t kk0 = 2 * (wave * n_pairs / 4);
    const int n_rows = (int)(2 * ((wave + 1) * n_pairs / 4) - kk0);
    const int64_t ld2 = a.ncol_pad;
    const d2* rows = reinterpret_cast<const d2*>(a.Bt) + kk0 * ld2 + cb * 64;
    double* strip = s_tiny + wave * strip_doubles;
    d2* part = reinterpret_cast<d2*>(s_tiny + 4 * strip_doubles);
    d2 buf0[GEMV_U], buf1[GEMV_U];
    auto fetch = [&](d2 (&buf)[GEMV_U], int base) {
#pragma unroll
        for (int u = 0; u < GEMV_U; ++u) buf[u] = rows[(int64_t)min(base + u, n_rows - 1) * ld2 + lane];
    };
    fetch(buf0, 0);
    fetch(buf1, GEMV_U);
    for (int rr = lane; rr < ((n_rows + 15) >> 4) * 8; rr += 64) {
        const int64_t r = (kk0 >> 1) + rr;
        double sn = 0.0, cs = 0.0;
        if (r < a.n_r && 2 * rr < n_rows) {
            double dot = 0.0;
            for (int d = 0; d < a.dim; ++d) dot = fma(hk_kcomp(a, 0, d), (double)a.R[r * a.dim + d], dot);
            sincospi(2.0 * dot, &sn, &cs);
        }
        strip[2 * rr] = cs;
        strip[2 * rr + 1] = sn;
    }
    asm volatile("s_waitcnt lgkmcnt(0)" ::: "memory");
    double acc0 = 0.0, acc1 = 0.0;
    auto consume = [&](const d2 (&buf)[GEMV_U], int row) {
#pragma unroll
        for (int u = 0; u < GEMV_U; ++u) {
            const double aq = strip[row + u];
            acc0 = fma(aq, buf[u][0], acc0);
            acc1 = fma(aq, buf[u][1], acc1);
        }
    };
    for (int row = 0; row < n_rows; row += 2 * GEMV_U) {
        consume(buf0, row);
        __builtin_amdgcn_sched_barrier(0);
        fetch(buf0, row + 2 * GEMV_U);
        __builtin_amdgcn_sched_barrier(0);
        consume(buf1, row + GEMV_U);
        __builtin_amdgcn_sched_barrier(0);
        fetch(buf1, row + 3 * GEMV_U);
        __builtin_amdgcn_sched_barrier(0);
    }
    const bool hi = (lane & 8) != 0;
    const int el = (lane >> 4) * 16 + (lane & 7) * 2 + (hi ? 1 : 0);
    const double got = __shfl_xor(hi ? acc0 : acc1, 8, 64);
    part[wave * 64 + el] = hi ? (d2){got, acc1} : (d2){acc0, got};
    __syncthreads();
    if (wave != 0) return;
    const int e = cb * 64 + lane;
    const int32_t ij = a.colmap[e];
    if (ij < 0) return;
    d2 sum = part[lane];
#pragma unroll
    for (int w = 1; w < 4; ++w) {
        sum[0] += part[w * 64 + lane][0];
        sum[1] += part[w * 64 + lane][1];
    }
    store_slot<MODE, CONV>(a, 0, ij, sum[0], sum[1]);
}

template <int MODE, int CONV>
__global__ void __launch_bounds__(256) hk_finish_kernel(const HkArgs a) {
    const int64_t idx = (int64_t)blockIdx.x * 256 + threadIdx.x;
    const int e = (int)(idx % a.ncol_pad);
    const int64_t kq = idx / a.ncol_pad;
    if (kq >= a.nk) return;
    const int32_t ij = a.colmap[e];
    if (ij < 0) return;
    double re = 0.0, im = 0.0;
    for (int sp = 0; sp < a.splits; ++sp) {
        const d2 v = *reinterpret_cast<const d2*>(a.P + (((size_t)sp * a.p_rows + kq) * a.ncol_pad + e) * 2);
        re += v[0];
        im += v[1];
    }
    store_slot<MODE, CONV>(a, kq, ij, re, im);
}

template <int MODE, int CONV>
__global__ void __launch_bounds__(256) hk_finish_wide_kernel(const HkArgs a) {
    __shared__ double part[4][16][2];
    const int lane = threadIdx.x & 63, wave = threadIdx.x >> 6;
    const int el = lane & 15;
    const int j = wave * 4 + (lane >> 4);
    const int64_t idx = (int64_t)blockIdx.x * 16 + el;
    const int e = (int)(idx % a.ncol_pad);
    const int64_t kq = idx / a.ncol_pad;
    double re = 0.0, im = 0.0;
    if (kq < a.nk)
        for (int sp = j; sp < a.splits; sp += 16) {
            const d2 v = *reinterpret_cast<const d2*>(a.P + (((size_t)sp * a.p_rows + kq) * a.ncol_pad + e) * 2);
            re += v[0];
            im += v[1];
        }
    re += __shfl_xor(re, 16, 64);
    im += __shfl_xor(im, 16, 64);
    re += __shfl_xor(re, 32, 64);
    im += __shfl_xor(im, 32, 64);
    if (lane < 16) {
        part[wave][el][0] = re;
        part[wave][el][1] = im;
    }
    __syncthreads();
    if (threadIdx.x < 16 && kq < a.nk) {
        const int32_t ij = a.colmap[e];
        if (ij < 0) return;
        const double sr = (part[0][el][0] + part[1][el][0]) + (part[2][el][0] + part[3][el][0]);
        const double si = (part[0][el][1] + part[1][el][1]) + (part[2][el][1] + part[3][el][1]);
        store_slot<MODE, CONV>(a, kq, ij, sr, si);
    }
}

template <int MODE, int CONV>
__global__ void __launch_bounds__(256) hk_finish_tiles_kernel(const HkArgs a) {
    const int unit = (int)blockIdx.x + a.block_offset;
    const int split_y = unit / a.unit_grid;
    int mt_idx, nt_idx;
    if (!tile_of_block(a, unit - split_y * a.unit_grid, mt_idx, nt_idx)) return;
    const int el = threadIdx.x & (TBK_BNP - 1);
    const int e = nt_idx * TBK_BNP + el;
    const int32_t ij = a.colmap[e];
    if (ij < 0) return;
    for (int local = threadIdx.x / TBK_BNP; local < a.rows_per_tile; local += 256 / TBK_BNP) {
        const int64_t kq = (int64_t)mt_idx * a.rows_per_tile + local;
        if (kq >= a.nk) break;
        double re = 0.0, im = 0.0;
        for (int sp = 0; sp < a.sub_splits; ++sp) {
            const d2 v = *reinterpret_cast<const d2*>(
                a.P2 + ((((size_t)sp * a.p_tiles + blockIdx.x) * TBK_BM + local) * TBK_BNP + el) * 2);
            re += v[0];
            im += v[1];
        }
        if (a.splits > 1)
            *reinterpret_cast<d2*>(a.P + (((size_t)split_y * a.p_rows + kq) * a.ncol_pad + e) * 2) = (d2){re, im};
        else
            store_slot<MODE, CONV>(a, kq, ij, re, im);
    }
}

template <int MODE, int CONV>
hipError_t launch_gemv(tbk_model* m, const HkArgs& a, size_t lds, hipStream_t s) {
    const int tasks = (a.ncol_pad >> 6) * a.splits;
    const dim3 grid((unsigned)((tasks + 3) / 4), 1, (unsigned)((a.nk + 31) / 32));
    static std::atomic<bool> raised[2][6][TBK_MAX_DEVICES] = {};
#define TBK_GEMV(N, SLOT)                                                                                               \
    do {                                                                                                                \
        if (a.A == nullptr) {                                                                                           \
            hipError_t e1 = tbk_raise_lds_limit(reinterpret_cast<const void*>(&hk_gemv_kernel<N, true>), 160 * 1024, raised[0][SLOT]); \
            if (e1 != hipSuccess) return e1;                                                                            \
            hipLaunchKernelGGL((hk_gemv_kernel<N, true>), grid, dim3(256), lds, s, a, (int)(lds / 32));                                  \
        } else {                                                                                                        \
            hipError_t e1 = tbk_raise_lds_limit(reinterpret_cast<const void*>(&hk_gemv_kernel<N, false>), 160 * 1024, raised[1][SLOT]); \
            if (e1 != hipSuccess) return e1;                                                                            \
            hipLaunchKernelGGL((hk_gemv_kernel<N, false>), grid, dim3(256), lds, s, a, (int)(lds / 32));                                 \
        }                                                                                                               \
    } while (0)
    if (a.nk <= 1)
        TBK_GEMV(1, 0);
    else if (a.nk <= 2)
        TBK_GEMV(2, 1);
    else if (a.nk <= 4)
        TBK_GEMV(4, 2);
    else if (a.nk <= 8)
        TBK_GEMV(8, 3);
    else if (a.nk <= 16)
        TBK_GEMV(16, 4);
    else
        TBK_GEMV(32, 5);
#undef TBK_GEMV
    (void)m;
    hipError_t e = hipGetLastError();
    if (e != hipSuccess) return e;
    const int64_t threads = a.nk * a.ncol_pad;
    if (a.splits >= 32)
        hipLaunchKernelGGL((hk_finish_wide_kernel<MODE, CONV>), dim3((unsigned)((threads + 15) / 16)), dim3(256), 0, s, a);
    else
        hipLaunchKernelGGL((hk_finish_kernel<MODE, CONV>), dim3((unsigned)((threads + 255) / 256)), dim3(256), 0, s, a);
    return hipGetLastError();
}

constexpr int TAIL_MAX_ROUNDS = 12;

template <int MODE, int CONV>
int launch(tbk_model* m, const HkArgs& a0, int grid) {
    hipStream_t s = m->stream;
    const size_t lds = 2 * STAGE_DOUBLES * sizeof(double);
    static std::atomic<bool> raised[TBK_MAX_DEVICES] = {};
    static std::atomic<bool> raised_split[TBK_MAX_DEVICES] = {};
    TBK_HIP(tbk_raise_lds_limit(reinterpret_cast<const void*>(&hk_dense_kernel<MODE, CONV, false>), 160 * 1024, raised));
    TBK_HIP(tbk_raise_lds_limit(reinterpret_cast<const void*>(&hk_dense_kernel<MODE, CONV, true>), 160 * 1024, raised_split));
    HkArgs a = a0;
    a.unit_grid = grid;
    const int slots = 2 * m->n_cu;
    const int n_stage = (int)(a.k2 / TBK_BK);
    const int units = grid * a.splits;
    const int full = units / slots * slots, tail = units - full;
    const int unit_stages = (n_stage + a.splits - 1) / a.splits;
    int sub = 1;
    if (full > 0 && tail > 0 && units < TAIL_MAX_ROUNDS * slots && unit_stages >= 8) {
        auto rounds = [&](int u) { return u <= slots / 2 ? 0.54 : (double)((u + slots - 1) / slots); };
        const double round_ms = 1.97 * unit_stages / 512.0;
        const double plain = rounds(tail) * round_ms;
        double best = std::min(0.9 * plain, plain - 0.03);
        for (int sp = 2; sp <= std::min(64, unit_stages / 4); ++sp) {
            const double cost = rounds(tail * sp) / sp * round_ms + sp * tail * 9e-5 + 0.01;
            if (cost < best) {
                best = cost;
                sub = sp;
            }
        }
    }
    const size_t base_bytes = a.splits > 1 ? (size_t)a.splits * a.p_rows * a.ncol_pad * 2 * sizeof(double) : 0;
    if (sub >= 2) {
        TBK_CHECK(m->ws_part.reserve(base_bytes + (size_t)sub * tail * TBK_BM * TBK_BNP * 2 * sizeof(double)));
        a.P = a.splits > 1 ? m->ws_part.as<double>() : nullptr;
        if (a.splits > 1)
            hipLaunchKernelGGL((hk_dense_kernel<MODE, CONV, true>), dim3(full), dim3(256), lds, s, a);
        else
            hipLaunchKernelGGL((hk_dense_kernel<MODE, CONV, false>), dim3(full), dim3(256), lds, s, a);
        TBK_HIP(hipGetLastError());
        HkArgs t = a;
        t.block_offset = full;
        t.p_tiles = tail;
        t.sub_splits = sub;
        t.P2 = reinterpret_cast<double*>(m->ws_part.as<char>() + base_bytes);
        hipLaunchKernelGGL((hk_dense_kernel<MODE, CONV, true>), dim3(tail, sub), dim3(256), lds, s, t);
        TBK_HIP(hipGetLastError());
        hipLaunchKernelGGL((hk_finish_tiles_kernel<MODE, CONV>), dim3(tail), dim3(256), 0, s, t);
        TBK_HIP(hipGetLastError());
    } else if (a.splits > 1) {
        hipLaunchKernelGGL((hk_dense_kernel<MODE, CONV, true>), dim3(units), dim3(256), lds, s, a);
        TBK_HIP(hipGetLastError());
    } else {
        hipLaunchKernelGGL((hk_dense_kernel<MODE, CONV, false>), dim3(grid), dim3(256), lds, s, a);
        TBK_HIP(hipGetLastError());
    }
    if (a.splits > 1) {
        const int64_t threads = a.nk * a.ncol_pad;
        hipLaunchKernelGGL((hk_finish_kernel<MODE, CONV>), dim3((unsigned)((threads + 255) / 256)), dim3(256), 0, s, a);
        TBK_HIP(hipGetLastError());
    }
    return TBK_OK;
}

int gemv_nkv(int64_t nk) {
    int nkv = 1;
    while (nkv < std::min<int64_t>(nk, 32)) nkv *= 2;
    return nkv;
}
int64_t gemv_strip_rows(const tbk_model* m, int64_t slices) {
    const int64_t n_pairs = m->k2 / 2;
    return (2 * ((n_pairs + slices - 1) / slices) + 15) / 16 * 16;
}

void gemv_plan(const tbk_model* m, int64_t nk, int* slices_out, size_t* lds_out) {
    const int nblk = m->ncol_pad / 64;
    const int64_t n_pairs = m->k2 / 2;
    const size_t per_split = (size_t)nk * m->ncol_pad * 2 * sizeof(double);
    const int64_t cap = std::max<int64_t>(1, (int64_t)((size_t(256) << 20) / per_split));
    const int64_t wave_slots = (int64_t)m->n_cu * 8;
    int64_t slices = wave_slots / nblk;
    size_t lds = 80 * 1024;
    const int64_t rows_one_round = slices > 0 ? (m->k2 + slices - 1) / slices : m->k2 + 1;
    if (slices < 1 || nblk * slices * 10 < wave_slots * 9 || rows_one_round > 384 || slices > cap) {
        slices = std::max<int64_t>(m->k2 / 256, std::min<int64_t>(((int64_t)m->n_cu * 32 + nblk - 1) / nblk, n_pairs / 8));
        slices = std::max<int64_t>(1, std::min(cap, slices));
        lds = 16 * 1024;
    }
    slices = std::max<int64_t>(1, std::min(slices, n_pairs / 8));
    if (nblk * slices * 2 <= wave_slots) lds = 16 * 1024;
    if (lds < 64 * 1024) {
        const size_t need = (size_t)4 * gemv_strip_rows(m, slices) * gemv_nkv(nk) * sizeof(double);
        if (need <= size_t(64) * 1024) lds = std::max(lds, need);
    }
    *slices_out = (int)slices;
    *lds_out = lds;
}

}

bool tbk_hk_inline_phases(const tbk_model* m, int64_t nk) {
    if (!tbk_hk_gemv_path(m, nk) || m->kdotp || m->d_R == nullptr) return false;
    int slices;
    size_t lds;
    gemv_plan(m, nk, &slices, &lds);
    return gemv_strip_rows(m, slices) * gemv_nkv(nk) <= (int64_t)(lds / 32);
}

bool tbk_hk_gemv_path(const tbk_model* m, int64_t nk) {
    if (nk < 1 || m->k2 <= 0 || m->sparse) return false;
    if (nk <= 32) return true;
    return nk <= 4096 && m->ncol_pad <= 256 && m->k2 < 16 * TBK_BK;
}

int tbk_launch_hk_dense(tbk_model* m, const double* d_A, int64_t nk, int64_t nk_pad, int mode,
                        int convention, const double* d_k, const double* d_pos, double* d_H) {
    if (nk == 0) return TBK_OK;
    HkArgs a;
    a.A = d_A;
    a.Bt = m->d_B;
    a.colmap = m->d_colmap;
    a.kpts = d_k;
    a.R = m->d_R;
    a.n_r = m->n_r;
    a.pos = d_pos;
    a.H = d_H;
    a.k2 = m->k2;
    a.nk = nk;
    a.nk_pad = nk_pad;
    a.ncol_pad = m->ncol_pad;
    a.n_orb = m->n_orb;
    a.dim = m->dim;
    a.mt_count = (int)((nk + TBK_BM - 1) / TBK_BM);
    a.nt_count = m->ncol_pad / TBK_BNP;
    int grid;
    if (a.mt_count >= 32) {
        a.xcd_rows = 4;
        const int max_rows = (a.mt_count + 7) / 8;
        grid = max_rows * a.nt_count * 8;
    } else {
        a.xcd_rows = 0;
        grid = a.mt_count * a.nt_count;
    }
    a.P = nullptr;
    a.splits = 1;
    a.p_rows = 0;
    a.a_tile_stride = TBK_BM;
    a.b_tile_stride = 0;
    a.rows_per_tile = TBK_BM;
    a.block_offset = 0;
    a.p_tiles = 0;
    a.sub_splits = 1;
    a.P2 = nullptr;
    a.unit_grid = 1;
    a.k_inline = 0;
    a.pos_raw = nullptr;
    for (int d = 0; d < TBK_MAX_DIM; ++d) a.k_val[d] = 0.0;
    if (tbk_hk_gemv_path(m, nk)) {
        int slices;
        size_t lds;
        gemv_plan(m, nk, &slices, &lds);
        const size_t per_split = (size_t)nk * a.ncol_pad * 2 * sizeof(double);
        if (m->h_k_inline != nullptr && nk == 1 && d_A == nullptr && tbk_hk_inline_phases(m, 1)) {
            a.k_inline = 1;
            for (int d = 0; d < m->dim; ++d) a.k_val[d] = m->h_k_inline[d];
            a.pos_raw = m->d_pos_inline;
        }
        TBK_ARG(d_A != nullptr || (tbk_hk_inline_phases(m, nk) && (d_k != nullptr || a.k_inline)), "phase rows missing");
        TBK_ARG(convention != 1 || mode == HK_TRI || d_pos != nullptr || (a.k_inline && a.pos_raw != nullptr), "convention 1 needs the orbital phases");
        if (nk == 1 && d_A == nullptr && a.ncol_pad <= 256 && m->k2 <= 4096) {
            const int strip = (int)(((m->k2 / 2 + 3) / 4 * 2 + 15) / 16 * 16);
            const size_t lds_tiny = ((size_t)4 * strip + 4 * 64 * 2) * sizeof(double);
            const dim3 grid_tiny((unsigned)(a.ncol_pad / 64));
            StageTimer t(m, TBK_T_HK);
            if (mode == HK_TRI)
                hipLaunchKernelGGL((hk_tiny_kernel<HK_TRI, 2>), grid_tiny, dim3(256), lds_tiny, m->stream, a, strip);
            else if (convention == 1)
                hipLaunchKernelGGL((hk_tiny_kernel<HK_FULL, 1>), grid_tiny, dim3(256), lds_tiny, m->stream, a, strip);
            else
                hipLaunchKernelGGL((hk_tiny_kernel<HK_FULL, 2>), grid_tiny, dim3(256), lds_tiny, m->stream, a, strip);
            TBK_HIP(hipGetLastError());
            return TBK_OK;
        }
        TBK_CHECK(m->ws_part.reserve(per_split * slices));
        a.P = m->ws_part.as<double>();
        a.splits = slices;
        a.p_rows = nk;
        StageTimer t(m, TBK_T_HK);
        if (mode == HK_TRI) {
            TBK_HIP((launch_gemv<HK_TRI, 2>(m, a, lds, m->stream)));
        } else if (convention == 1) {
            TBK_HIP((launch_gemv<HK_FULL, 1>(m, a, lds, m->stream)));
        } else {
            TBK_HIP((launch_gemv<HK_FULL, 2>(m, a, lds, m->stream)));
        }
        return TBK_OK;
    }
    const int n_stage = (int)(m->k2 / TBK_BK);
    const int tiles = a.mt_count * a.nt_count;
    if (tiles < 2 * m->n_cu && n_stage >= 16) {
        int splits = std::min((1280 + tiles / 2) / tiles, n_stage / 4);
        const size_t per_split = (size_t)nk_pad * a.ncol_pad * 2 * sizeof(double);
        splits = (int)std::min<size_t>((size_t)splits, (size_t(512) << 20) / per_split);
        if (splits > 1) {
            TBK_CHECK(m->ws_part.reserve(per_split * splits));
            a.P = m->ws_part.as<double>();
            a.splits = splits;
            a.p_rows = nk_pad;
        }
    }
    StageTimer t(m, TBK_T_HK);
    if (mode == HK_TRI) {
        TBK_CHECK((launch<HK_TRI, 2>(m, a, grid)));
    } else if (convention == 1) {
        TBK_CHECK((launch<HK_FULL, 1>(m, a, grid)));
    } else {
        TBK_CHECK((launch<HK_FULL, 2>(m, a, grid)));
    }
    return TBK_OK;
}

int tbk_launch_hk_dense_lines(tbk_model* m, const double* d_A, int64_t n_lines, int line_len, int64_t b_stride,
                              double* d_H) {
    if (n_lines == 0) return TBK_OK;
    TBK_ARG(line_len >= 1 && line_len <= TBK_BM, "a mesh line must fit one k tile");
    HkArgs a;
    a.A = d_A;
    a.Bt = m->d_B;
    a.colmap = m->d_colmap;
    a.kpts = nullptr;
    a.R = m->d_R;
    a.n_r = m->n_r;
    a.pos = nullptr;
    a.H = d_H;
    a.k2 = m->k2;
    a.nk = n_lines * line_len;
    a.nk_pad = TBK_BM;
    a.ncol_pad = m->ncol_pad;
    a.n_orb = m->n_orb;
    a.dim = m->dim;
    a.mt_count = (int)n_lines;
    a.nt_count = m->ncol_pad / TBK_BNP;
    a.P = nullptr;
    a.splits = 1;
    a.p_rows = 0;
    a.a_tile_stride = 0;
    a.b_tile_stride = b_stride;
    a.rows_per_tile = line_len;
    a.block_offset = 0;
    a.p_tiles = 0;
    a.sub_splits = 1;
    a.P2 = nullptr;
    a.unit_grid = 1;
    int grid;
    if (a.mt_count >= 32) {
        a.xcd_rows = 4;
        grid = ((a.mt_count + 7) / 8) * a.nt_count * 8;
    } else {
        a.xcd_rows = 0;
        grid = a.mt_count * a.nt_count;
    }
    StageTimer t(m, TBK_T_HK);
    TBK_CHECK((launch<HK_TRI, 2>(m, a, grid)));
    return TBK_OK;
}
```

### tbmodels_amd/csrc/tbk_internal.h

```cpp
#pragma once

#include <hip/hip_runtime.h>
#include <rocblas/rocblas.h>

#include <atomic>
#include <cstdlib>
#include <cstdint>
#include <cstdio>
#include <functional>
#include <mutex>
#include <string>
#include <vector>

#include "tbk.h"

constexpr int TBK_BM = 128;
constexpr int TBK_BNP = 64;
constexpr int TBK_BK = 16;
constexpr int TBK_CT = 16;
constexpr int TBK_MAX_DIM = 8;

constexpr int32_t TBK_SLOT_PAIR = 0x8000;

void tbk_set_error(const char* fmt, ...);

#define TBK_HIP(expr)                                                                             \
    do {                                                                                          \
        hipError_t e_ = (expr);                                                                   \
        if (e_ != hipSuccess) {                                                                   \
            tbk_set_error("%s failed: %s (%s:%d)", #expr, hipGetErrorString(e_), __FILE__,        \
                          __LINE__);                                                              \
            return (e_ == hipErrorOutOfMemory) ? TBK_ERR_MEMORY : TBK_ERR_DEVICE;                 \
        }                                                                                         \
    } while (0)

#define TBK_ROCBLAS(expr)                                                                         \
    do {                                                                                          \
        rocblas_status s_ = (expr);                                                               \
        if (s_ != rocblas_status_success) {                                                       \
            tbk_set_error("%s failed: rocblas_status %d (%s:%d)", #expr, (int)s_, __FILE__,       \
                          __LINE__);                                                              \
            return (s_ == rocblas_status_memory_error) ? TBK_ERR_MEMORY : TBK_ERR_DEVICE;         \
        }                                                                                         \
    } while (0)

#define TBK_CHECK(expr)                                                                           \
    do {                                                                                          \
        int r_ = (expr);                                                                          \
        if (r_ != TBK_OK) return r_;                                                              \
    } while (0)

#define TBK_LOCK(m) std::lock_guard<std::recursive_mutex> tbk_lock_((m)->mu)

#define TBK_ARG(cond, msg)                                                                        \
    do {                                                                                          \
        if (!(cond)) {                                                                            \
            tbk_set_error("invalid argument: %s", msg);                                           \
            return TBK_ERR_ARGUMENT;                                                              \
        }                                                                                         \
    } while (0)


constexpr int TBK_MAX_DEVICES = 64;

using tbk_flag_row = std::atomic<bool>[TBK_MAX_DEVICES];
inline hipError_t tbk_raise_lds_limit(const void* kernel, int bytes, tbk_flag_row& done) {
    int dev = 0;
    hipError_t e = hipGetDevice(&dev);
    if (e != hipSuccess) return e;
    if (dev >= 0 && dev < TBK_MAX_DEVICES && done[dev].load(std::memory_order_acquire)) return hipSuccess;
    e = hipFuncSetAttribute(kernel, hipFuncAttributeMaxDynamicSharedMemorySize, bytes);
    if (e == hipSuccess && dev >= 0 && dev < TBK_MAX_DEVICES) done[dev].store(true, std::memory_order_release);
    return e;
}

struct DevBuf {
    void* ptr = nullptr;
    size_t bytes = 0;
    int reserve(size_t want);
    void release();
    template <class T>
    T* as() const {
        return static_cast<T*>(ptr);
    }
};

struct EventPair {
    hipEvent_t start, stop;
    int stage;
};

struct tbk_fold_plan_t {
    bool built = false;
    int dim = 0;
    int64_t n_r = 0;
    int64_t n_rho = 0, n_rho_pad = 0, k2 = 0;
    int capacity = 0;
    std::vector<int32_t> h_R2;
    int32_t* d_R2 = nullptr;
    int64_t* d_lptr = nullptr;
    int32_t* d_lrec = nullptr;
    int32_t* d_rcomp = nullptr;
    double* d_B2 = nullptr;
    double* d_table = nullptr;
    int64_t table_entries = 0;
    tbk_fold_plan_t* sub = nullptr;
};

struct tbk_fold_saved_t {
    int dim;
    int64_t n_r, n_r_pad, k2;
    int32_t* d_R;
    double* d_B;
};

struct tbk_model {
    std::recursive_mutex mu;
    int device = 0;
    int64_t call_nk = 0;
    int n_cu = 256;
    int dim = 0;
    int n_orb = 0;
    int64_t n_r = 0;
    bool sparse = false;
    bool kdotp = false;

    int64_t n_r_pad = 0;
    int64_t k2 = 0;
    int ncol = 0;
    int ncol_pad = 0;
    int32_t* d_R = nullptr;
    int32_t* d_colmap = nullptr;
    int32_t* d_powers = nullptr;

    double* d_B = nullptr;

    int64_t nnz_rec = 0;
    int64_t* d_cptr = nullptr;
    int32_t* d_rec_r = nullptr;
    double* d_rec_v = nullptr;
    int sched_kt = 0;
    int64_t sched_steps = 0;
    int64_t* d_sptr = nullptr;
    int32_t* d_srec_r = nullptr;
    double* d_srec_v = nullptr;

    int64_t staged_bytes = 0;

    std::vector<int32_t> h_R;
    tbk_fold_plan_t fold[TBK_MAX_DIM];
    bool fold_enabled = true;
    int64_t counters[TBK_CNT_COUNT] = {0, 0, 0, 0};

    int eigensolver = TBK_EIG_AUTO;
    int64_t k_chunk = 0;
    bool timing = false;

    hipStream_t stream = nullptr;
    hipStream_t stream_eig = nullptr;
    hipStream_t stream_ql = nullptr;
    hipStream_t stream_xl[3] = {nullptr, nullptr, nullptr};
    hipEvent_t ev_xl[4] = {nullptr, nullptr, nullptr, nullptr};
    hipEvent_t ev_hk[2] = {nullptr, nullptr};
    hipEvent_t ev_tri[2] = {nullptr, nullptr};
    hipEvent_t ev_out[2] = {nullptr, nullptr};
    hipEvent_t ev_ql[2] = {nullptr, nullptr};
    hipEvent_t ev_sync = nullptr;
    rocblas_handle blas = nullptr;
    DevBuf ws_phase;
    DevBuf ws_H;
    DevBuf ws_H2;
    DevBuf ws_E;
    DevBuf ws_E2;
    DevBuf ws_info;
    DevBuf ws_k;
    DevBuf ws_pos;
    DevBuf ws_orb;
    DevBuf ws_out;
    DevBuf ws_out2;
    DevBuf ws_flag;
    void* h_stage = nullptr;
    size_t h_stage_bytes = 0;
    DevBuf ws_part;
    DevBuf ws_kfold;
    DevBuf ws_kline;
    DevBuf ws_band;
    DevBuf ws_bandmat[2];
    const double* h_k_inline = nullptr;
    const double* d_pos_inline = nullptr;
    std::vector<double> pos_cache;
    DevBuf ws_posraw;
    DevBuf ws_xl;
    std::function<int(int64_t c0, int64_t nkc, hipEvent_t done)> chunk_done;
    std::vector<EventPair> events;
    double t_ms[TBK_T_COUNT] = {0, 0, 0, 0};
    int64_t t_n[TBK_T_COUNT] = {0, 0, 0, 0};
};

struct tbk_kdotp {
    tbk_model* core = nullptr;
};

void tbk_range_push(const char* name);
void tbk_range_pop();

struct StageTimer {
    tbk_model* m;
    EventPair ev;
    bool on;
    hipStream_t stream;
    StageTimer(tbk_model* m_, int stage, hipStream_t s = nullptr);
    ~StageTimer();
};

enum HkMode { HK_TRI = 0, HK_FULL = 1 };

int tbk_launch_phase(tbk_model* m, const double* d_k, int64_t nk, int64_t nk_pad, double* d_A);
int tbk_launch_orbital_phases(tbk_model* m, const double* d_k, const double* d_pos, int64_t nk, double* d_orb);
int tbk_launch_monomials(hipStream_t s, const int32_t* d_powers, int dim, int64_t n_p,
                         int64_t n_p_pad, const double* d_k, int64_t nk, int64_t nk_pad,
                         double* d_A);

int tbk_stage_dense(tbk_model* m, const double* d_hop_raw);
int tbk_stage_kdotp(tbk_model* m, const double* d_coeff_raw);

int tbk_launch_hk_dense(tbk_model* m, const double* d_A, int64_t nk, int64_t nk_pad, int mode,
                        int convention, const double* d_k, const double* d_pos, double* d_H);

int tbk_launch_hk_dense_lines(tbk_model* m, const double* d_A, int64_t n_lines, int line_len, int64_t b_stride, double* d_H);

int tbk_launch_hk_csr(tbk_model* m, const double* d_A, int64_t nk, int64_t nk_pad, int mode,
                      int convention, const double* d_k, const double* d_pos, double* d_H);

int tbk_csr_tile_kpoints(int64_t n_r);
void tbk_csr_schedule(int ncol, int kt, const std::vector<int64_t>& cptr, const std::vector<int32_t>& rec_r, const std::vector<double>& rec_v,
                      std::vector<int64_t>& sptr, std::vector<int32_t>& srec_r, std::vector<double>& srec_v);

int tbk_eig_batched(tbk_model* m, double* d_H, int64_t nk, double* d_E);

bool tbk_eig_stream_supported(int n);
int tbk_launch_tridiag_stream(tbk_model* m, hipStream_t s, double* d_H, int64_t nk, double* d_de, int method = 0);
bool tbk_hk_inline_phases(const tbk_model* m, int64_t nk);
bool tbk_hk_gemv_path(const tbk_model* m, int64_t nk);
int tbk_launch_bisect(tbk_model* m, hipStream_t s, const double* d_de, int64_t nk, double* d_E);
size_t tbk_eig_scratch_per_k(const tbk_model* m);
int tbk_band_xl_reserve(tbk_model* m, int64_t max_nk);

bool tbk_eig_band_supported(int n);
bool tbk_eig_band_preferred(int n);
size_t tbk_band_scratch_per_matrix(int n);
size_t tbk_band_bytes_per_matrix(int n);
size_t tbk_band_xl_buffer_per_matrix(int n);
bool tbk_eig_two_stage(const tbk_model* m);
int tbk_launch_band_reduce(tbk_model* m, hipStream_t s, double* d_H, int64_t nk, void* d_vw, void* d_band,
                           double* d_de_fused = nullptr);
bool tbk_band_fused(int n);
bool tbk_band_split(const tbk_model* m, int64_t nk);
bool tbk_band_xl_grouped(int n, int64_t nk);
int tbk_launch_band_chase(tbk_model* m, hipStream_t s, const void* d_band, int64_t nk, double* d_de);

bool tbk_eig_small_supported(int n);
int tbk_launch_tridiag(tbk_model* m, hipStream_t s, double* d_H, int64_t nk, double* d_de);
bool tbk_eig_reg128_supported(int n);
int tbk_launch_tridiag_reg128(hipStream_t s, double* d_H, int n, int64_t nk, double* d_D, double* d_E, int64_t h_stride, int ldd, int off);
int tbk_launch_tridiag_tail64(hipStream_t s, double* d_H, int64_t nk, double* d_D, double* d_E, int n_full, int64_t call_nk);
int tbk_launch_ql(tbk_model* m, hipStream_t s, const double* d_de, int64_t nk, double* d_E, bool beside_ql = false);

int tbk_fold_choose(tbk_model* m, const double* h_k, int64_t nk, std::vector<int64_t>& run_starts);
int tbk_fold_group_size();
int tbk_fold_group(tbk_model* m, tbk_fold_plan_t& plan, const double* h_kf, int n_g, int slot0);
int tbk_fold_lines(tbk_model* m, tbk_fold_plan_t& plan, const double* d_kf, int64_t stride, int n_lines, int slot0 = 0);
int tbk_fold_enter(tbk_model* m, tbk_fold_plan_t& plan, int slot, tbk_fold_saved_t& saved);
void tbk_fold_leave(tbk_model* m, const tbk_fold_saved_t& saved);
int tbk_fold_drop_component(tbk_model* m, const double* d_k, int dim, int f, int64_t nk, double* d_k2);
int tbk_fold_subplan(tbk_model* m, tbk_fold_plan_t& parent, int f2, int capacity, tbk_fold_plan_t** out);
void tbk_fold_release(tbk_model* m);
int64_t tbk_fold_min_run();

int tbk_run_mfma_f64_peak(double* tflops);
```

### tbmodels_amd/csrc/tbk_phase.hip

```cpp

#include "tbk_internal.h"

namespace {

__global__ void __launch_bounds__(256)
phase_rows_kernel(const double* __restrict__ k, const int32_t* __restrict__ R, int dim, int64_t nk,
                  int64_t nk_pad, int64_t n_r, double* __restrict__ A) {
    const int64_t kidx = (int64_t)blockIdx.x * blockDim.x + threadIdx.x;
    const int64_t r = blockIdx.y;
    if (kidx >= nk_pad) return;
    double c = 0.0, s = 0.0;
    if (kidx < nk && r < n_r) {
        double dot = 0.0;
        for (int d = 0; d < dim; ++d)
            dot = fma(k[kidx * dim + d], (double)R[r * dim + d], dot);
        sincospi(2.0 * dot, &s, &c);
    }
    A[(2 * r) * nk_pad + kidx] = c;
    A[(2 * r + 1) * nk_pad + kidx] = s;
}

__global__ void __launch_bounds__(256)
monomial_rows_kernel(const double* __restrict__ k, const int32_t* __restrict__ powers, int dim,
                     int64_t nk, int64_t nk_pad, int64_t n_p, double* __restrict__ A) {
    const int64_t kidx = (int64_t)blockIdx.x * blockDim.x + threadIdx.x;
    const int64_t p = blockIdx.y;
    if (kidx >= nk_pad) return;
    double v = 0.0;
    if (kidx < nk && p < n_p) {
        v = 1.0;
        for (int d = 0; d < dim; ++d) {
            const double x = k[kidx * dim + d];
            const int e = powers[p * dim + d];
            double acc = 1.0;
            for (int t = 0; t < e; ++t) acc *= x;
            v *= acc;
        }
    }
    A[p * nk_pad + kidx] = v;
}

__global__ void __launch_bounds__(256)
orbital_phase_kernel(const double* __restrict__ k, const double* __restrict__ pos, int dim, int64_t nk,
                     int n_orb, double* __restrict__ orb) {
    const int64_t idx = (int64_t)blockIdx.x * blockDim.x + threadIdx.x;
    if (idx >= nk * n_orb) return;
    const int64_t kq = idx / n_orb;
    const int p = (int)(idx % n_orb);
    double dot = 0.0;
    for (int d = 0; d < dim; ++d) dot = fma(k[kq * dim + d], pos[p * dim + d], dot);
    double s, c;
    sincospi(2.0 * dot, &s, &c);
    orb[2 * idx] = c;
    orb[2 * idx + 1] = s;
}

}

int tbk_launch_orbital_phases(tbk_model* m, const double* d_k, const double* d_pos, int64_t nk, double* d_orb) {
    if (nk == 0) return TBK_OK;
    const int64_t total = nk * m->n_orb;
    hipLaunchKernelGGL(orbital_phase_kernel, dim3((unsigned)((total + 255) / 256)), dim3(256), 0, m->stream, d_k,
                       d_pos, m->dim, nk, m->n_orb, d_orb);
    TBK_HIP(hipGetLastError());
    return TBK_OK;
}

int tbk_launch_phase(tbk_model* m, const double* d_k, int64_t nk, int64_t nk_pad, double* d_A) {
    if (m->n_r_pad == 0 || nk_pad == 0) return TBK_OK;
    StageTimer t(m, TBK_T_PHASE);
    dim3 grid((unsigned)((nk_pad + 255) / 256), (unsigned)m->n_r_pad);
    hipLaunchKernelGGL(phase_rows_kernel, grid, dim3(256), 0, m->stream, d_k, m->d_R, m->dim, nk,
                       nk_pad, m->n_r, d_A);
    TBK_HIP(hipGetLastError());
    return TBK_OK;
}

int tbk_launch_monomials(hipStream_t s, const int32_t* d_powers, int dim, int64_t n_p,
                         int64_t n_p_pad, const double* d_k, int64_t nk, int64_t nk_pad,
                         double* d_A) {
    if (n_p_pad == 0 || nk_pad == 0) return TBK_OK;
    dim3 grid((unsigned)((nk_pad + 255) / 256), (unsigned)n_p_pad);
    hipLaunchKernelGGL(monomial_rows_kernel, grid, dim3(256), 0, s, d_k, d_powers, dim, nk, nk_pad,
                       n_p, d_A);
    TBK_HIP(hipGetLastError());
    return TBK_OK;
}
```

### tbmodels_amd/csrc/tbk_stage.hip

```cpp

#include "tbk_internal.h"

namespace {

__global__ void __launch_bounds__(256)
stage_dense_kernel(const double* __restrict__ hop, const int32_t* __restrict__ colmap, int n_orb,
                   int64_t n_r, int ncol_pad, double* __restrict__ Bt) {
    const int e = blockIdx.x * blockDim.x + threadIdx.x;
    const int64_t r = blockIdx.y;
    if (e >= ncol_pad || r >= n_r) return;
    const int32_t ij = colmap[e];
    if (ij < 0) return;
    const int i = ij >> 16, j = ij & 0x7fff;
    const double* blk = hop + (size_t)r * n_orb * n_orb * 2;
    const size_t tiles = ncol_pad / TBK_CT;
    const size_t base0 = (((size_t)(2 * r) * tiles + e / TBK_CT) * 2) * TBK_CT + e % TBK_CT;
    const size_t base1 = (((size_t)(2 * r + 1) * tiles + e / TBK_CT) * 2) * TBK_CT + e % TBK_CT;
    if (ij & TBK_SLOT_PAIR) {
        const double hr = blk[((size_t)i * n_orb + i) * 2], hi = blk[((size_t)i * n_orb + i) * 2 + 1];
        const double gr = blk[((size_t)j * n_orb + j) * 2], gi = blk[((size_t)j * n_orb + j) * 2 + 1];
        Bt[base0] = hr + hr;
        Bt[base0 + TBK_CT] = gr + gr;
        Bt[base1] = -(hi + hi);
        Bt[base1 + TBK_CT] = -(gi + gi);
        return;
    }
    const double hr = blk[((size_t)i * n_orb + j) * 2], hi = blk[((size_t)i * n_orb + j) * 2 + 1];
    const double gr = blk[((size_t)j * n_orb + i) * 2], gi = blk[((size_t)j * n_orb + i) * 2 + 1];
    Bt[base0] = hr + gr;
    Bt[base0 + TBK_CT] = hi - gi;
    Bt[base1] = -(hi + gi);
    Bt[base1 + TBK_CT] = hr - gr;
}

__global__ void __launch_bounds__(256)
stage_kdotp_kernel(const double* __restrict__ coeff, const int32_t* __restrict__ colmap, int n_orb,
                   int64_t n_p, int ncol_pad, double* __restrict__ Bt) {
    const int e = blockIdx.x * blockDim.x + threadIdx.x;
    const int64_t p = blockIdx.y;
    if (e >= ncol_pad || p >= n_p) return;
    const int32_t ij = colmap[e];
    if (ij < 0) return;
    const int i = ij >> 16, j = ij & 0xffff;
    const double* blk = coeff + (size_t)p * n_orb * n_orb * 2;
    const size_t tiles = ncol_pad / TBK_CT;
    const size_t base = (((size_t)p * tiles + e / TBK_CT) * 2) * TBK_CT + e % TBK_CT;
    Bt[base] = blk[((size_t)i * n_orb + j) * 2];
    Bt[base + TBK_CT] = blk[((size_t)i * n_orb + j) * 2 + 1];
}

}

int tbk_stage_dense(tbk_model* m, const double* d_hop_raw) {
    const size_t bytes = (size_t)m->k2 * m->ncol_pad * 2 * sizeof(double);
    if (bytes == 0) return TBK_OK;
    TBK_HIP(hipMalloc((void**)&m->d_B, bytes));
    m->staged_bytes += (int64_t)bytes;
    TBK_HIP(hipMemsetAsync(m->d_B, 0, bytes, m->stream));
    if (m->n_r > 0) {
        TBK_ARG(m->n_r <= 65535, "more than 65535 lattice vectors");
        dim3 grid((m->ncol_pad + 255) / 256, (unsigned)m->n_r);
        hipLaunchKernelGGL(stage_dense_kernel, grid, dim3(256), 0, m->stream, d_hop_raw, m->d_colmap,
                           m->n_orb, m->n_r, m->ncol_pad, m->d_B);
        TBK_HIP(hipGetLastError());
    }
    return TBK_OK;
}

int tbk_stage_kdotp(tbk_model* m, const double* d_coeff_raw) {
    const size_t bytes = (size_t)m->k2 * m->ncol_pad * 2 * sizeof(double);
    if (bytes == 0) return TBK_OK;
    TBK_HIP(hipMalloc((void**)&m->d_B, bytes));
    m->staged_bytes += (int64_t)bytes;
    TBK_HIP(hipMemsetAsync(m->d_B, 0, bytes, m->stream));
    if (m->n_r > 0) {
        TBK_ARG(m->n_r <= 65535, "more than 65535 Taylor coefficients");
        dim3 grid((m->ncol_pad + 255) / 256, (unsigned)m->n_r);
        hipLaunchKernelGGL(stage_kdotp_kernel, grid, dim3(256), 0, m->stream, d_coeff_raw,
                           m->d_colmap, m->n_orb, m->n_r, m->ncol_pad, m->d_B);
        TBK_HIP(hipGetLastError());
    }
    return TBK_OK;
}
```

Measured before the change: 988,600 k-points/s.

## Compute H(k) GEMM with int8 MFMA via multi-modulus residue arithmetic

Adds an Ozaki/CRT-style path for the dense H(k) build. Phases and staged hoppings are quantized to fixed-point integers and split into several int8 residues. The product is then computed with int8 MFMA per modulus and reconstructed in double precision by a finish kernel that uses a Horner-style sum. A certification step at staging decides whether error bounds permit the path, and chunk sizing accounts for the extra residue buffers. The aim is to replace the f64 GEMM with much higher-throughput int8 matrix ops. In exchange it adds extra memory traffic, a reconstruction kernel and quantization error bounded by the certificate.

Measured after the change: 1.067 million k-points/s (median of 6 runs). 1.08x the previous value.

```diff
diff --git a/include/tbk.h b/include/tbk.h
--- a/include/tbk.h
+++ b/include/tbk.h
@@ -46,7 +46,8 @@
                    int* is_sparse, int64_t* staged_bytes);
 enum { TBK_CNT_EIGENVAL_CALLS = 0, TBK_CNT_FOLDED_CALLS = 1, TBK_CNT_FOLDED_KPOINTS = 2,
        TBK_CNT_LIBRARY_CALLS = 3,
-       TBK_CNT_COUNT = 4 };
+       TBK_CNT_INT8_KPOINTS = 4,
+       TBK_CNT_COUNT = 5 };
 int tbk_model_counter(tbk_model* m, int counter, int64_t* value);
 
 
diff --git a/tbmodels_amd/csrc/tbk_api.hip b/tbmodels_amd/csrc/tbk_api.hip
--- a/tbmodels_amd/csrc/tbk_api.hip
+++ b/tbmodels_amd/csrc/tbk_api.hip
@@ -233,6 +233,7 @@
             TBK_HIP(hipMemcpyAsync(d_raw, hop, raw_bytes, hipMemcpyHostToDevice, m->stream));
         }
         TBK_CHECK(tbk_stage_dense(m, d_raw));
+        TBK_CHECK(tbk_stage_i8(m));
         TBK_HIP(hipStreamSynchronize(m->stream));
         return TBK_OK;
     }();
@@ -352,11 +353,11 @@
     if (m->h_stage) (void)hipHostFree(m->h_stage);
     for (hipStream_t st : streams)
         if (st) (void)hipStreamDestroy(st);
-    void* ptrs[] = {m->d_R, m->d_colmap, m->d_B, m->d_cptr, m->d_rec_r, m->d_rec_v, m->d_powers, m->d_sptr, m->d_srec_r, m->d_srec_v};
+    void* ptrs[] = {m->d_R, m->d_colmap, m->d_B, m->d_B8, m->d_i8_scale, m->d_cptr, m->d_rec_r, m->d_rec_v, m->d_powers, m->d_sptr, m->d_srec_r, m->d_srec_v};
     for (void* p : ptrs)
         if (p) (void)hipFree(p);
     DevBuf* bufs[] = {&m->ws_phase, &m->ws_H, &m->ws_E,   &m->ws_E2,
-                      &m->ws_info,  &m->ws_k, &m->ws_pos, &m->ws_out, &m->ws_out2, &m->ws_flag, &m->ws_orb, &m->ws_part, &m->ws_kfold, &m->ws_kline, &m->ws_band, &m->ws_bandmat[0], &m->ws_bandmat[1], &m->ws_H2, &m->ws_xl, &m->ws_posraw};
+                      &m->ws_info,  &m->ws_k, &m->ws_pos, &m->ws_out, &m->ws_out2, &m->ws_flag, &m->ws_orb, &m->ws_part, &m->ws_kfold, &m->ws_kline, &m->ws_band, &m->ws_bandmat[0], &m->ws_bandmat[1], &m->ws_H2, &m->ws_xl, &m->ws_posraw, &m->ws_phase8, &m->ws_res8};
     for (DevBuf* b : bufs) b->release();
     tbk_fold_release(m);
     delete m;
@@ -398,18 +399,33 @@
     return TBK_OK;
 }
 
-static int64_t choose_chunk(tbk_model* m, int64_t nk, bool with_eig) {
-    if (nk <= TBK_BM) return TBK_BM;
+static int64_t choose_chunk(tbk_model* m, int64_t nk, bool with_eig, bool direct = true) {
+    if (nk <= TBK_BM) {
+        m->i8_call = m->i8_ok;
+        return TBK_BM;
+    }
     const int64_t n = m->n_orb;
     int64_t per_k = m->k2 * 8 + (with_eig ? n * n * 16 + (int64_t)tbk_eig_scratch_per_k(m) : 0);
+
     if (per_k < 64) per_k = 64;
     size_t free_b = 0, total_b = 0;
     if (hipMemGetInfo(&free_b, &total_b) != hipSuccess) free_b = size_t(8) << 30;
     free_b += m->ws_H.bytes + m->ws_H2.bytes + m->ws_phase.bytes + m->ws_band.bytes + m->ws_bandmat[0].bytes + m->ws_bandmat[1].bytes +
-              m->ws_E.bytes + m->ws_xl.bytes;
+              m->ws_E.bytes + m->ws_xl.bytes + m->ws_phase8.bytes + m->ws_res8.bytes;
     const bool mid = n > 64 && n <= 256;
     int64_t budget = std::min<int64_t>((int64_t)(free_b / 4), int64_t(mid ? 64 : n > 64 ? 24 : 6) << 30);
     int64_t chunk = budget / per_k / TBK_BM * TBK_BM;
+    m->i8_call = false;
+    if (m->i8_ok && direct && m->k_chunk == 0) {
+        const int64_t per_k8 = per_k + (int64_t)TBK_I8_NMOD * (m->k2 + 2 * m->ncol_pad) - m->k2 * 8;
+        const int64_t chunk8 = budget / per_k8 / TBK_BM * TBK_BM;
+        if (chunk8 >= tbk_i8_min_nk() || (chunk8 >= TBK_BM && round_up(nk, TBK_BM) <= chunk8)) {
+            chunk = chunk8;
+            m->i8_call = true;
+        }
+    } else if (m->i8_ok && direct) {
+        m->i8_call = true;
+    }
     int64_t cap = mid ? 131072 : 32768;
     if (n < 64) cap *= std::min<int64_t>(32, (64 / n) * (64 / n));
     chunk = std::max<int64_t>(TBK_BM, std::min<int64_t>(chunk, cap));
@@ -421,6 +437,10 @@
 static inline int64_t phase_ld(int64_t nk) { return round_up(nk, TBK_BM); }
 
 static int fill_rows(tbk_model* m, const double* d_k, int64_t nk, int64_t nk_pad, double* d_A) {
+    if (tbk_hk_i8_path(m, nk)) {
+        TBK_CHECK(m->ws_phase8.reserve((size_t)TBK_I8_NMOD * nk_pad * m->k2));
+        return tbk_launch_phase_i8(m, d_k, nk, nk_pad, m->ws_phase8.as<int8_t>());
+    }
     if (m->kdotp)
         return tbk_launch_monomials(m->stream, m->d_powers, m->dim, m->n_r, m->k2, d_k, nk, nk_pad, d_A);
     return tbk_launch_phase(m, d_k, nk, nk_pad, d_A);
@@ -448,7 +468,7 @@
     for (int64_t c0 = 0; c0 < nk; c0 += chunk) {
         const int64_t nkc = std::min(chunk, nk - c0);
         const int64_t nk_pad = phase_ld(nkc);
-        TBK_CHECK(m->ws_phase.reserve((size_t)std::max<int64_t>(m->k2, 1) * nk_pad * sizeof(double)));
+        if (!tbk_hk_i8_path(m, nkc)) TBK_CHECK(m->ws_phase.reserve((size_t)std::max<int64_t>(m->k2, 1) * nk_pad * sizeof(double)));
         double* d_A = m->ws_phase.as<double>();
         const double* kc = d_k + c0 * m->dim;
         const bool own_rows = tbk_hk_inline_phases(m, nkc);
@@ -522,7 +542,7 @@
     const auto prepare_rows = [&](int64_t c0, int64_t nkc) -> int {
         if (tbk_hk_inline_phases(m, nkc)) return TBK_OK;
         const int64_t nk_pad = phase_ld(nkc);
-        TBK_CHECK(m->ws_phase.reserve((size_t)std::max<int64_t>(m->k2, 1) * nk_pad * sizeof(double)));
+        if (!tbk_hk_i8_path(m, nkc)) TBK_CHECK(m->ws_phase.reserve((size_t)std::max<int64_t>(m->k2, 1) * nk_pad * sizeof(double)));
         TBK_CHECK(fill_rows(m, d_k + c0 * m->dim, nkc, nk_pad, m->ws_phase.as<double>()));
         rows_ready_for = c0;
         return TBK_OK;
@@ -535,7 +555,7 @@
         return build_h(m, m->ws_phase.as<double>(), nkc, nk_pad, HK_TRI, 2, kc, nullptr, d_H);
     };
     const HBuilder& build = builder ? *builder : direct;
-    const int64_t chunk = choose_chunk(m, nk, true);
+    const int64_t chunk = choose_chunk(m, nk, true, builder == nullptr);
     const size_t n = (size_t)m->n_orb;
     const size_t nn2 = n * n * 2;
     DevBuf* debuf[2] = {&m->ws_E, &m->ws_E2};
@@ -649,7 +669,7 @@
 
     auto piece_plane = [&](int64_t lo, int64_t hi, double* d_Hp) -> int {
         const int64_t len = hi - lo, nk_pad = phase_ld(len);
-        TBK_CHECK(m->ws_phase.reserve((size_t)std::max<int64_t>(m->k2, 1) * nk_pad * sizeof(double)));
+        if (!tbk_hk_i8_path(m, len)) TBK_CHECK(m->ws_phase.reserve((size_t)std::max<int64_t>(m->k2, 1) * nk_pad * sizeof(double)));
         TBK_CHECK(fill_rows(m, d_k2 + lo * (dim - 1), len, nk_pad, m->ws_phase.as<double>()));
         return build_h(m, m->ws_phase.as<double>(), len, nk_pad, HK_TRI, 2, d_k2 + lo * (dim - 1), nullptr, d_Hp);
     };
@@ -847,7 +867,7 @@
     for (int64_t c0 = 0; c0 < nk; c0 += chunk) {
         const int64_t nkc = std::min(chunk, nk - c0);
         const int64_t nk_pad = phase_ld(nkc);
-        TBK_CHECK(m->ws_phase.reserve((size_t)std::max<int64_t>(m->k2, 1) * nk_pad * sizeof(double)));
+        if (!tbk_hk_i8_path(m, nkc)) TBK_CHECK(m->ws_phase.reserve((size_t)std::max<int64_t>(m->k2, 1) * nk_pad * sizeof(double)));
         TBK_CHECK(m->ws_H.reserve((size_t)nkc * nn2 * sizeof(double)));
         double* d_A = m->ws_phase.as<double>();
         double* d_H = m->ws_H.as<double>();
diff --git a/tbmodels_amd/csrc/tbk_hk_dense.hip b/tbmodels_amd/csrc/tbk_hk_dense.hip
--- a/tbmodels_amd/csrc/tbk_hk_dense.hip
+++ b/tbmodels_amd/csrc/tbk_hk_dense.hip
@@ -95,7 +95,8 @@
     store_element<MODE, CONV>(a, kq, oi, oj, v0, v1);
 }
 
-__device__ __forceinline__ bool tile_of_block(const HkArgs& a, int b, int& mt, int& nt) {
+template <class Args>
+__device__ __forceinline__ bool tile_of_block(const Args& a, int b, int& mt, int& nt) {
     if (a.xcd_rows == 0) {
         nt = b % a.nt_count;
         mt = b / a.nt_count;
@@ -621,6 +622,210 @@
     return TBK_OK;
 }
 
+typedef int i4 __attribute__((ext_vector_type(4)));
+constexpr int I8_BM = TBK_BM;
+constexpr int I8_BN = 2 * TBK_BNP;
+constexpr int I8_BK = 64;
+static_assert(I8_BM == 128 && I8_BN == 128, "wave decomposition is written for 128 x 128");
+
+struct I8Args {
+    const int8_t* A8;
+    const int8_t* B8;
+    uint8_t* R8;
+    int64_t k2;
+    int64_t nk_pad;
+    int64_t ncol2;
+    int mt_count, nt_count, xcd_rows, tiles_grid;
+    int mod[TBK_I8_NMOD];
+};
+
+__global__ void __launch_bounds__(256) hk_i8_kernel(const I8Args a) {
+    __shared__ __attribute__((aligned(16))) int8_t smem[2][(I8_BM + I8_BN) * I8_BK];
+    const int mod = (int)blockIdx.x / a.tiles_grid;
+    int mt, nt;
+    if (!tile_of_block(a, (int)blockIdx.x - mod * a.tiles_grid, mt, nt)) return;
+    const int lane = threadIdx.x & 63;
+    const int wave = __builtin_amdgcn_readfirstlane(threadIdx.x >> 6);
+    const int wm = wave >> 1, wn = wave & 1;
+    const int64_t k2 = a.k2;
+    const int8_t* gA = a.A8 + ((int64_t)mod * a.nk_pad + (int64_t)mt * I8_BM + 32 * wave) * k2;
+    const int8_t* gB = a.B8 + ((int64_t)mod * a.ncol2 + (int64_t)nt * I8_BN + 32 * wave) * k2;
+    const uint32_t src = (uint32_t)(lane >> 2) * (uint32_t)k2 + 16u * (uint32_t)((lane & 3) ^ ((lane >> 4) & 3));
+    auto issue = [&](int buf, int st) {
+        int8_t* sA = &smem[buf][0] + 32 * wave * I8_BK;
+        int8_t* sB = &smem[buf][I8_BM * I8_BK] + 32 * wave * I8_BK;
+        const int64_t koff = (int64_t)st * I8_BK;
+        uint32_t off = src;
+        asm volatile("" : "+v"(off));
+#pragma unroll
+        for (int h = 0; h < 2; ++h) {
+            __builtin_amdgcn_global_load_lds((gptr_t)(gA + h * 16 * k2 + koff + off), (lptr_t)(sA + h * 16 * I8_BK), 16, 0, 0);
+            __builtin_amdgcn_global_load_lds((gptr_t)(gB + h * 16 * k2 + koff + off), (lptr_t)(sB + h * 16 * I8_BK), 16, 0, 0);
+        }
+    };
+    const int fr = (lane & 15) * I8_BK + 16 * ((lane >> 4) ^ ((lane >> 2) & 3));
+    const int offA = wm * 64 * I8_BK + fr;
+    const int offB = I8_BM * I8_BK + wn * 64 * I8_BK + fr;
+
+    i4 acc[4][4];
+#pragma unroll
+    for (int i = 0; i < 4; ++i)
+#pragma unroll
+        for (int j = 0; j < 4; ++j) acc[i][j] = (i4){0, 0, 0, 0};
+    const int n_stage = (int)(k2 / I8_BK);
+    issue(0, 0);
+    for (int st = 0; st < n_stage; ++st) {
+        const int buf = st & 1;
+        __syncthreads();
+        if (st + 1 < n_stage) issue(buf ^ 1, st + 1);
+        const int8_t* sb = &smem[buf][0];
+        i4 fa[4], fb[4];
+#pragma unroll
+        for (int i = 0; i < 4; ++i) {
+            fa[i] = *reinterpret_cast<const i4*>(sb + offA + i * 16 * I8_BK);
+            fb[i] = *reinterpret_cast<const i4*>(sb + offB + i * 16 * I8_BK);
+        }
+#pragma unroll
+        for (int i = 0; i < 4; ++i)
+#pragma unroll
+            for (int j = 0; j < 4; ++j) acc[i][j] = __builtin_amdgcn_mfma_i32_16x16x64_i8(fa[i], fb[j], acc[i][j], 0, 0, 0);
+    }
+    const int mi = a.mod[mod];
+    const double inv = 1.0 / (double)mi;
+    uint8_t* out = a.R8 + ((int64_t)mod * a.nk_pad + (int64_t)mt * I8_BM) * a.ncol2 + (int64_t)nt * I8_BN;
+#pragma unroll
+    for (int i = 0; i < 4; ++i)
+#pragma unroll
+        for (int j = 0; j < 4; ++j)
+#pragma unroll
+            for (int r = 0; r < 4; ++r) {
+                const int row = wm * 64 + i * 16 + 4 * (lane >> 4) + r, col = wn * 64 + j * 16 + (lane & 15);
+                int v = acc[i][j][r];
+                v -= (int)rint((double)v * inv) * mi;
+                if (v < 0) v += mi;
+                out[(int64_t)row * a.ncol2 + col] = (uint8_t)v;
+            }
+}
+
+struct I8Fin {
+    const uint8_t* R8;
+    const double* scale;
+    int64_t plane;
+    int64_t ncol2;
+    float m[TBK_I8_NMOD], inv[TBK_I8_NMOD], hi[TBK_I8_NMOD], lo[TBK_I8_NMOD];
+    float c[TBK_I8_NMOD][TBK_I8_NMOD];
+};
+
+typedef float f2 __attribute__((ext_vector_type(2)));
+
+__device__ __forceinline__ double i8_horner(const float (&v)[TBK_I8_NMOD], const I8Fin& f) {
+    double sh = (double)v[TBK_I8_NMOD - 1], sl = 0.0;
+#pragma unroll
+    for (int i = TBK_I8_NMOD - 2; i >= 0; --i) {
+        const double mm = (double)f.m[i], vi = (double)v[i];
+        const double ph = sh * mm, pl = fma(sl, mm, fma(sh, mm, -ph));
+        const double th = ph + vi, bb = th - ph, te = (ph - (th - bb)) + (vi - bb);
+        const double tl = te + pl;
+        sh = th + tl;
+        const double b2 = sh - th;
+        sl = (th - (sh - b2)) + (tl - b2);
+    }
+    return sh;
+}
+
+template <int MODE, int CONV>
+__global__ void __launch_bounds__(256) hk_i8_finish_kernel(const HkArgs a, const I8Fin f) {
+    const int e0 = 4 * ((int)blockIdx.x * 256 + (int)threadIdx.x);
+    if (e0 >= a.ncol_pad) return;
+    const int64_t c0 = 32 * (e0 >> 4) + (e0 & 15);
+    int32_t ij[4];
+#pragma unroll
+    for (int t = 0; t < 4; ++t) ij[t] = a.colmap[e0 + t];
+    if (ij[0] < 0 && ij[1] < 0 && ij[2] < 0 && ij[3] < 0) return;
+    constexpr float MAGIC = 12582912.0f;
+    for (int64_t kq = blockIdx.y; kq < a.nk; kq += gridDim.y) {
+        const uint8_t* p = f.R8 + kq * f.ncol2 + c0;
+        uint32_t wr[TBK_I8_NMOD], wi[TBK_I8_NMOD];
+#pragma unroll
+        for (int i = 0; i < TBK_I8_NMOD; ++i) {
+            wr[i] = *reinterpret_cast<const uint32_t*>(p + i * f.plane);
+            wi[i] = *reinterpret_cast<const uint32_t*>(p + 16 + i * f.plane);
+        }
+#pragma unroll
+        for (int t = 0; t < 4; ++t) {
+            if (ij[t] < 0) continue;
+            float vr[TBK_I8_NMOD], vim[TBK_I8_NMOD];
+#pragma unroll
+            for (int i = 0; i < TBK_I8_NMOD; ++i) {
+                f2 y = (f2){(float)((wr[i] >> (8 * t)) & 255u), (float)((wi[i] >> (8 * t)) & 255u)};
+#pragma unroll
+                for (int j = 0; j < i; ++j) {
+                    y = (y - (f2){vr[j], vim[j]}) * f.c[j][i];
+                    const f2 q = (y * f.inv[i] + MAGIC) - MAGIC;
+                    y = y - q * f.m[i];
+                }
+                vr[i] = y.x > f.hi[i] ? y.x - f.m[i] : (y.x < f.lo[i] ? y.x + f.m[i] : y.x);
+                vim[i] = y.y > f.hi[i] ? y.y - f.m[i] : (y.y < f.lo[i] ? y.y + f.m[i] : y.y);
+            }
+            const double re = i8_horner(vr, f) * f.scale[c0 + t], im = i8_horner(vim, f) * f.scale[c0 + 16 + t];
+            store_slot<MODE, CONV>(a, kq, ij[t], re, im);
+        }
+    }
+}
+
+int inv_mod(int x, int m) {
+    int t = 0, nt = 1, r = m, nr = x % m;
+    while (nr) {
+        const int q = r / nr;
+        int tmp = t - q * nt;
+        t = nt;
+        nt = tmp;
+        tmp = r - q * nr;
+        r = nr;
+        nr = tmp;
+    }
+    return t < 0 ? t + m : t;
+}
+
+template <int MODE, int CONV>
+int launch_i8(tbk_model* m, const HkArgs& a, int grid) {
+    const int64_t ncol2 = 2 * (int64_t)a.ncol_pad;
+    const int64_t plane = a.nk_pad * ncol2;
+    TBK_CHECK(m->ws_res8.reserve((size_t)TBK_I8_NMOD * plane));
+    I8Args g;
+    g.A8 = m->ws_phase8.as<int8_t>();
+    g.B8 = m->d_B8;
+    g.R8 = m->ws_res8.as<uint8_t>();
+    g.k2 = a.k2;
+    g.nk_pad = a.nk_pad;
+    g.ncol2 = ncol2;
+    g.mt_count = a.mt_count;
+    g.nt_count = a.nt_count;
+    g.xcd_rows = a.xcd_rows;
+    g.tiles_grid = grid;
+    I8Fin f;
+    f.R8 = g.R8;
+    f.scale = m->d_i8_scale;
+    f.plane = plane;
+    f.ncol2 = ncol2;
+    for (int i = 0; i < TBK_I8_NMOD; ++i) {
+        const int mi = m->i8_mod[i];
+        g.mod[i] = mi;
+        f.m[i] = (float)mi;
+        f.inv[i] = 1.0f / (float)mi;
+        f.hi[i] = (float)((mi - 1) / 2);
+        f.lo[i] = (float)(-(mi / 2));
+        for (int j = 0; j < TBK_I8_NMOD; ++j) f.c[j][i] = j < i ? (float)inv_mod(m->i8_mod[j] % mi, mi) : 0.0f;
+    }
+    hipStream_t s = m->stream;
+    hipLaunchKernelGGL(hk_i8_kernel, dim3((unsigned)(grid * TBK_I8_NMOD)), dim3(256), 0, s, g);
+    TBK_HIP(hipGetLastError());
+    const dim3 fin((unsigned)((a.ncol_pad / 4 + 255) / 256), (unsigned)std::min<int64_t>(a.nk, 65535));
+    hipLaunchKernelGGL((hk_i8_finish_kernel<MODE, CONV>), fin, dim3(256), 0, s, a, f);
+    TBK_HIP(hipGetLastError());
+    return TBK_OK;
+}
+
 int gemv_nkv(int64_t nk) {
     int nkv = 1;
     while (nkv < std::min<int64_t>(nk, 32)) nkv *= 2;
@@ -669,6 +874,14 @@
     if (nk < 1 || m->k2 <= 0 || m->sparse) return false;
     if (nk <= 32) return true;
     return nk <= 4096 && m->ncol_pad <= 256 && m->k2 < 16 * TBK_BK;
+}
+
+constexpr int64_t TBK_I8_MIN_NK = 4096;
+
+int64_t tbk_i8_min_nk() { return TBK_I8_MIN_NK; }
+
+bool tbk_hk_i8_path(const tbk_model* m, int64_t nk) {
+    return m->i8_ok && m->i8_call && m->d_B == m->i8_src && m->d_B8 != nullptr && nk >= TBK_I8_MIN_NK && m->k2 % I8_BK == 0 && !tbk_hk_gemv_path(m, nk);
 }
 
 int tbk_launch_hk_dense(tbk_model* m, const double* d_A, int64_t nk, int64_t nk_pad, int mode,
@@ -751,6 +964,19 @@
             TBK_HIP((launch_gemv<HK_FULL, 1>(m, a, lds, m->stream)));
         } else {
             TBK_HIP((launch_gemv<HK_FULL, 2>(m, a, lds, m->stream)));
+        }
+        return TBK_OK;
+    }
+    if (tbk_hk_i8_path(m, nk)) {
+        TBK_ARG(convention != 1 || mode == HK_TRI || d_pos != nullptr, "convention 1 needs the orbital phases");
+        m->counters[TBK_CNT_INT8_KPOINTS] += nk;
+        StageTimer t(m, TBK_T_HK);
+        if (mode == HK_TRI) {
+            TBK_CHECK((launch_i8<HK_TRI, 2>(m, a, grid)));
+        } else if (convention == 1) {
+            TBK_CHECK((launch_i8<HK_FULL, 1>(m, a, grid)));
+        } else {
+            TBK_CHECK((launch_i8<HK_FULL, 2>(m, a, grid)));
         }
         return TBK_OK;
     }
diff --git a/tbmodels_amd/csrc/tbk_i8_cert.h b/tbmodels_amd/csrc/tbk_i8_cert.h
--- /dev/null
+++ b/tbmodels_amd/csrc/tbk_i8_cert.h
@@ -0,0 +1,61 @@
+#pragma once
+
+#include <algorithm>
+#include <cmath>
+#include <cstdint>
+#include <vector>
+
+constexpr int TBK_I8_A = 53;
+constexpr int TBK_I8_NMOD = 16;
+
+struct tbk_i8_cert {
+    int mod[TBK_I8_NMOD];
+    double log2p;
+    double bound_rel;
+    int bmin, bmax;
+};
+
+inline bool tbk_i8_certify(const std::vector<double>& norm1, int64_t k_rows, std::vector<int>& b, tbk_i8_cert& cert) {
+    if (k_rows <= 0 || k_rows >= (int64_t(1) << 17)) return false;
+    int kk = 0;
+    while ((int64_t(1) << kk) < k_rows) ++kk;
+    int n = 0;
+    double log2p = 0.0;
+    for (int m = 256; m >= 2 && n < TBK_I8_NMOD; --m) {
+        bool ok = true;
+        for (int i = 0; i < n && ok; ++i) {
+            int x = m, y = cert.mod[i];
+            while (y) {
+                const int t = x % y;
+                x = y;
+                y = t;
+            }
+            ok = x == 1;
+        }
+        if (!ok) continue;
+        cert.mod[n++] = m;
+        log2p += std::log2((double)m);
+    }
+    cert.log2p = log2p;
+    if (log2p < TBK_I8_A + 58 + kk) return false;
+    b.assign(norm1.size(), 0);
+    bool any = false;
+    cert.bmin = 1 << 30;
+    cert.bmax = -(1 << 30);
+    cert.bound_rel = 0.0;
+    for (size_t c = 0; c < norm1.size(); ++c) {
+        const double s = norm1[c];
+        if (!std::isfinite(s)) return false;
+        if (s == 0.0) continue;
+        any = true;
+        const int e = std::ilogb(s * (1.0 - 0x1p-30));
+        const int bc = TBK_I8_A + 1 + kk - e;
+        if (TBK_I8_A + bc > 1020 || TBK_I8_A + bc < -1000) return false;
+        b[c] = bc;
+        cert.bmin = std::min(cert.bmin, bc);
+        cert.bmax = std::max(cert.bmax, bc);
+        const double bound = 0x1p-54 + (double)k_rows * std::ldexp(1.0, -(bc + 1)) * (1.0 + 0x1p-54) / (s * (1.0 - 0x1p-30));
+        cert.bound_rel = std::max(cert.bound_rel, bound);
+    }
+    return any && cert.bound_rel <= 0x1p-53;
+}
diff --git a/tbmodels_amd/csrc/tbk_internal.h b/tbmodels_amd/csrc/tbk_internal.h
--- a/tbmodels_amd/csrc/tbk_internal.h
+++ b/tbmodels_amd/csrc/tbk_internal.h
@@ -13,6 +13,7 @@
 #include <vector>
 
 #include "tbk.h"
+#include "tbk_i8_cert.h"
 
 constexpr int TBK_BM = 128;
 constexpr int TBK_BNP = 64;
@@ -21,6 +22,7 @@
 constexpr int TBK_MAX_DIM = 8;
 
 constexpr int32_t TBK_SLOT_PAIR = 0x8000;
+
 
 void tbk_set_error(const char* fmt, ...);
 
@@ -145,12 +147,22 @@
     int32_t* d_srec_r = nullptr;
     double* d_srec_v = nullptr;
 
+    bool i8_ok = false;
+    bool i8_call = true;
+    const double* i8_src = nullptr;
+    int8_t* d_B8 = nullptr;
+    double* d_i8_scale = nullptr;
+    int i8_mod[TBK_I8_NMOD] = {};
+    double i8_bound_rel = 0.0;
+    int i8_bmin = 0, i8_bmax = 0;
+    double i8_log2p = 0.0;
+
     int64_t staged_bytes = 0;
 
     std::vector<int32_t> h_R;
     tbk_fold_plan_t fold[TBK_MAX_DIM];
     bool fold_enabled = true;
-    int64_t counters[TBK_CNT_COUNT] = {0, 0, 0, 0};
+    int64_t counters[TBK_CNT_COUNT] = {0, 0, 0, 0, 0};
 
     int eigensolver = TBK_EIG_AUTO;
     int64_t k_chunk = 0;
@@ -181,6 +193,8 @@
     DevBuf ws_flag;
     void* h_stage = nullptr;
     size_t h_stage_bytes = 0;
+    DevBuf ws_phase8;
+    DevBuf ws_res8;
     DevBuf ws_part;
     DevBuf ws_kfold;
     DevBuf ws_kline;
@@ -217,12 +231,14 @@
 
 int tbk_launch_phase(tbk_model* m, const double* d_k, int64_t nk, int64_t nk_pad, double* d_A);
 int tbk_launch_orbital_phases(tbk_model* m, const double* d_k, const double* d_pos, int64_t nk, double* d_orb);
+int tbk_launch_phase_i8(tbk_model* m, const double* d_k, int64_t nk, int64_t nk_pad, int8_t* d_A8);
 int tbk_launch_monomials(hipStream_t s, const int32_t* d_powers, int dim, int64_t n_p,
                          int64_t n_p_pad, const double* d_k, int64_t nk, int64_t nk_pad,
                          double* d_A);
 
 int tbk_stage_dense(tbk_model* m, const double* d_hop_raw);
 int tbk_stage_kdotp(tbk_model* m, const double* d_coeff_raw);
+int tbk_stage_i8(tbk_model* m);
 
 int tbk_launch_hk_dense(tbk_model* m, const double* d_A, int64_t nk, int64_t nk_pad, int mode,
                         int convention, const double* d_k, const double* d_pos, double* d_H);
@@ -242,6 +258,8 @@
 int tbk_launch_tridiag_stream(tbk_model* m, hipStream_t s, double* d_H, int64_t nk, double* d_de, int method = 0);
 bool tbk_hk_inline_phases(const tbk_model* m, int64_t nk);
 bool tbk_hk_gemv_path(const tbk_model* m, int64_t nk);
+bool tbk_hk_i8_path(const tbk_model* m, int64_t nk);
+int64_t tbk_i8_min_nk();
 int tbk_launch_bisect(tbk_model* m, hipStream_t s, const double* d_de, int64_t nk, double* d_E);
 size_t tbk_eig_scratch_per_k(const tbk_model* m);
 int tbk_band_xl_reserve(tbk_model* m, int64_t max_nk);
diff --git a/tbmodels_amd/csrc/tbk_phase.hip b/tbmodels_amd/csrc/tbk_phase.hip
--- a/tbmodels_amd/csrc/tbk_phase.hip
+++ b/tbmodels_amd/csrc/tbk_phase.hip
@@ -1,3 +1,5 @@
+
+#include <algorithm>
 
 #include "tbk_internal.h"
 
@@ -18,6 +20,45 @@
     }
     A[(2 * r) * nk_pad + kidx] = c;
     A[(2 * r + 1) * nk_pad + kidx] = s;
+}
+
+struct ModArgs {
+    double m[TBK_I8_NMOD], inv[TBK_I8_NMOD];
+};
+__global__ void __launch_bounds__(256)
+phase_i8_kernel(const double* __restrict__ k, const int32_t* __restrict__ R, int dim, int64_t nk, int64_t nk_pad, int64_t n_r,
+                int64_t n_r_pad, const ModArgs ma, int8_t* __restrict__ A8) {
+    const int64_t r0 = ((int64_t)blockIdx.x * blockDim.x + threadIdx.x) * 8;
+    if (r0 >= n_r_pad) return;
+    const int64_t k2 = 2 * n_r_pad;
+    for (int64_t kidx = blockIdx.y; kidx < nk_pad; kidx += gridDim.y) {
+        double x[16];
+#pragma unroll
+        for (int t = 0; t < 8; ++t) {
+            const int64_t r = r0 + t;
+            double c = 0.0, s = 0.0;
+            if (kidx < nk && r < n_r) {
+                double dot = 0.0;
+                for (int d = 0; d < dim; ++d) dot = fma(k[kidx * dim + d], (double)R[r * dim + d], dot);
+                sincospi(2.0 * dot, &s, &c);
+            }
+            x[2 * t] = rint(ldexp(c, TBK_I8_A));
+            x[2 * t + 1] = rint(ldexp(s, TBK_I8_A));
+        }
+#pragma unroll
+        for (int i = 0; i < TBK_I8_NMOD; ++i) {
+            const int mi = (int)ma.m[i];
+            uint32_t w[4] = {0u, 0u, 0u, 0u};
+#pragma unroll
+            for (int t = 0; t < 16; ++t) {
+                int v = (int)fma(-rint(x[t] * ma.inv[i]), ma.m[i], x[t]);
+                if (v > (mi - 1) / 2) v -= mi;
+                if (v < -(mi / 2)) v += mi;
+                w[t >> 2] |= (uint32_t)(uint8_t)(int8_t)v << (8 * (t & 3));
+            }
+            *reinterpret_cast<uint4*>(A8 + ((size_t)i * nk_pad + kidx) * k2 + 2 * r0) = make_uint4(w[0], w[1], w[2], w[3]);
+        }
+    }
 }
 
 __global__ void __launch_bounds__(256)
@@ -76,6 +117,20 @@
     return TBK_OK;
 }
 
+int tbk_launch_phase_i8(tbk_model* m, const double* d_k, int64_t nk, int64_t nk_pad, int8_t* d_A8) {
+    if (m->n_r_pad == 0 || nk_pad == 0) return TBK_OK;
+    StageTimer t(m, TBK_T_PHASE);
+    ModArgs ma;
+    for (int i = 0; i < TBK_I8_NMOD; ++i) {
+        ma.m[i] = (double)m->i8_mod[i];
+        ma.inv[i] = 1.0 / ma.m[i];
+    }
+    dim3 grid((unsigned)((m->n_r_pad / 8 + 255) / 256), (unsigned)std::min<int64_t>(nk_pad, 65535));
+    hipLaunchKernelGGL(phase_i8_kernel, grid, dim3(256), 0, m->stream, d_k, m->d_R, m->dim, nk, nk_pad, m->n_r, m->n_r_pad, ma, d_A8);
+    TBK_HIP(hipGetLastError());
+    return TBK_OK;
+}
+
 int tbk_launch_monomials(hipStream_t s, const int32_t* d_powers, int dim, int64_t n_p,
                          int64_t n_p_pad, const double* d_k, int64_t nk, int64_t nk_pad,
                          double* d_A) {
diff --git a/tbmodels_amd/csrc/tbk_stage.hip b/tbmodels_amd/csrc/tbk_stage.hip
--- a/tbmodels_amd/csrc/tbk_stage.hip
+++ b/tbmodels_amd/csrc/tbk_stage.hip
@@ -1,3 +1,5 @@
+
+#include <cmath>
 
 #include "tbk_internal.h"
 
@@ -49,6 +51,92 @@
     Bt[base + TBK_CT] = blk[((size_t)i * n_orb + j) * 2 + 1];
 }
 
+__global__ void __launch_bounds__(256) column_norm1_kernel(const double* __restrict__ Bt, int64_t k2, int ncol2, double* __restrict__ norm1) {
+    const int c = blockIdx.x * blockDim.x + threadIdx.x;
+    if (c >= ncol2) return;
+    double s = 0.0;
+    for (int64_t kk = 0; kk < k2; ++kk) s += fabs(Bt[kk * ncol2 + c]);
+    norm1[c] = s;
+}
+
+struct ModTable {
+    int mod[TBK_I8_NMOD];
+};
+__global__ void __launch_bounds__(256) stage_i8_kernel(const double* __restrict__ Bt, int64_t k2, int ncol2, const int* __restrict__ bexp,
+                                                       const ModTable mt, int8_t* __restrict__ B8) {
+    const int64_t kk = (int64_t)blockIdx.x * blockDim.x + threadIdx.x;
+    const int c = blockIdx.y;
+    if (kk >= k2) return;
+    const double x = rint(ldexp(Bt[kk * ncol2 + c], bexp[c]));
+#pragma unroll
+    for (int i = 0; i < TBK_I8_NMOD; ++i) {
+        const int mi = mt.mod[i];
+        int r = (int)fmod(x, (double)mi);
+        if (r > (mi - 1) / 2) r -= mi;
+        if (r < -(mi / 2)) r += mi;
+        B8[((size_t)i * ncol2 + c) * k2 + kk] = (int8_t)r;
+    }
+}
+
+}
+
+int tbk_stage_i8(tbk_model* m) {
+    m->i8_ok = false;
+    if (m->sparse || m->kdotp || m->d_B == nullptr || m->n_r == 0) return TBK_OK;
+    const int ncol2 = 2 * m->ncol_pad;
+    const size_t res_bytes = (size_t)TBK_I8_NMOD * ncol2 * m->k2;
+    const int64_t per_k8 = (int64_t)TBK_I8_NMOD * (m->k2 + (int64_t)ncol2);
+    if (per_k8 * tbk_i8_min_nk() > (int64_t(6) << 30)) return TBK_OK;
+    size_t free_b = 0, total_b = 0;
+    if (hipMemGetInfo(&free_b, &total_b) != hipSuccess || res_bytes > free_b / 4) return TBK_OK;
+    double* d_norm = nullptr;
+    int* d_b = nullptr;
+    std::vector<double> norm1(ncol2);
+    TBK_HIP(hipMalloc((void**)&d_norm, ncol2 * sizeof(double)));
+    hipLaunchKernelGGL(column_norm1_kernel, dim3((ncol2 + 255) / 256), dim3(256), 0, m->stream, m->d_B, m->k2, ncol2, d_norm);
+    hipError_t e = hipGetLastError();
+    if (e == hipSuccess) e = hipMemcpyAsync(norm1.data(), d_norm, ncol2 * sizeof(double), hipMemcpyDeviceToHost, m->stream);
+    if (e == hipSuccess) e = hipStreamSynchronize(m->stream);
+    (void)hipFree(d_norm);
+    TBK_HIP(e);
+    std::vector<int> b;
+    tbk_i8_cert cert;
+    if (!tbk_i8_certify(norm1, 2 * m->n_r, b, cert)) return TBK_OK;
+    std::vector<double> scale(ncol2);
+    for (int c = 0; c < ncol2; ++c) scale[c] = std::ldexp(1.0, -(TBK_I8_A + b[c]));
+    auto give_up = [&]() -> int {
+        (void)hipGetLastError();
+        if (m->d_B8) (void)hipFree(m->d_B8);
+        if (m->d_i8_scale) (void)hipFree(m->d_i8_scale);
+        if (d_b) (void)hipFree(d_b);
+        m->d_B8 = nullptr;
+        m->d_i8_scale = nullptr;
+        return TBK_OK;
+    };
+    if (hipMalloc((void**)&m->d_B8, res_bytes) != hipSuccess || hipMalloc((void**)&m->d_i8_scale, ncol2 * sizeof(double)) != hipSuccess ||
+        hipMalloc((void**)&d_b, ncol2 * sizeof(int)) != hipSuccess)
+        return give_up();
+    ModTable mt;
+    for (int i = 0; i < TBK_I8_NMOD; ++i) mt.mod[i] = cert.mod[i];
+    e = hipMemcpyAsync(d_b, b.data(), ncol2 * sizeof(int), hipMemcpyHostToDevice, m->stream);
+    if (e == hipSuccess) e = hipMemcpyAsync(m->d_i8_scale, scale.data(), ncol2 * sizeof(double), hipMemcpyHostToDevice, m->stream);
+    if (e == hipSuccess) {
+        hipLaunchKernelGGL(stage_i8_kernel, dim3((unsigned)((m->k2 + 255) / 256), (unsigned)ncol2), dim3(256), 0, m->stream, m->d_B, m->k2,
+                           ncol2, d_b, mt, m->d_B8);
+        e = hipGetLastError();
+    }
+    if (e == hipSuccess) e = hipStreamSynchronize(m->stream);
+    if (e != hipSuccess) return give_up();
+    (void)hipFree(d_b);
+    m->staged_bytes += (int64_t)(res_bytes + ncol2 * sizeof(double));
+    for (int i = 0; i < TBK_I8_NMOD; ++i) m->i8_mod[i] = cert.mod[i];
+    m->i8_bound_rel = cert.bound_rel;
+    m->i8_bmin = cert.bmin;
+    m->i8_bmax = cert.bmax;
+    m->i8_log2p = cert.log2p;
+    m->i8_src = m->d_B;
+    m->i8_ok = true;
+    return TBK_OK;
 }
 
 int tbk_stage_dense(tbk_model* m, const double* d_hop_raw) {
```
